# Lukeasargen/Show-Attend-and-Tell-Pytorch-Lightning

Hardware: AMD Instinct MI355X
Metric: captions/sec (train step) at B=128, 256px, seq_len=22 (higher is better)
Workload: dtype bf16; 1 GPU; C2: resnet50 encoder_size=7 encoder_dim=512 vocab=6400 T=22, 128 images/GPU x R=5 captions, trainable encoder, Adam, full lengths, decoder_tf=always; global_batch_images=128, parallelism=dp1, grad_bucket_dtype=fp32

## Files before the change

### include/sat_hip.h

```cpp
#ifndef SAT_HIP_H
#define SAT_HIP_H
#include <stddef.h>
#include <stdint.h>

#ifdef __cplusplus
extern "C" {
#endif

#define SAT_HIP_ABI_VERSION 23

int sat_abi_version(void);
int sat_debug_trace_launches(int32_t on);
int sat_debug_option(const char* name, int32_t value);
const char* sat_last_error(void);

typedef struct sat_profile_entry {
    char name[96];
    int64_t launches;
    double total_ms;
    double flops;
    double bytes;
} sat_profile_entry;
int sat_profile_start(void);
int sat_profile_start_only(const char* name);
int sat_profile_pause(int32_t paused);
int sat_profile_stop(sat_profile_entry* out, int32_t max_entries, int32_t* n_out);

typedef struct sat_gemm_desc {
    const float* A; int64_t lda; const int32_t* a_rows;
    const float* B; int64_t ldb;
    float* C; int64_t ldc;       const int32_t* c_rows;
    int32_t M, N, K;
    int32_t amode, bmode;
    int32_t accumulate;
    int32_t epi;
    const float* bias; const float* e0; int64_t lde0; int32_t c0, c1;
    float* slab; int64_t slab_elems;
} sat_gemm_desc;
int sat_gemm_f32(const sat_gemm_desc* d, void* stream);
typedef struct sat_gemm_types { int32_t a_bf16, b_bf16, c_bf16, bf16_mfma; } sat_gemm_types;
int sat_gemm_ex(const sat_gemm_desc* d, const sat_gemm_types* t, void* stream);

typedef struct sat_decoder_dims {
    int32_t B;
    int32_t R;
    int32_t T;
    int32_t L;
    int32_t D;
    int32_t A;
    int32_t m;
    int32_t n;
    int32_t V;
    int32_t P;
    int32_t deep_output;
    int32_t padding_idx;
    int32_t precision;
    int32_t layers;
    float embed_max_norm;
    float dropout;
    float embedding_dropout;
    uint64_t dropout_seed;
} sat_decoder_dims;

#define SAT_MAX_LSTM_LAYERS 4
typedef struct sat_decoder_params {
    float* embedding;
    float* init_f_w; float* init_f_b;
    float* init_i_w; float* init_i_b;
    float* w_ih; float* w_hh;
    float* b_ih; float* b_hh;
    float* att_enc;
    float* att_dec;
    float* att_f;
    float* beta_w; float* beta_b;
    float* out_hidden;
    float* out_context;
    float* out_w; float* out_b;
    float* up_w_ih[SAT_MAX_LSTM_LAYERS - 1]; float* up_w_hh[SAT_MAX_LSTM_LAYERS - 1];
    float* up_b_ih[SAT_MAX_LSTM_LAYERS - 1]; float* up_b_hh[SAT_MAX_LSTM_LAYERS - 1];
} sat_decoder_params;

typedef struct sat_decoder_batch {
    const float* ann;
    const int32_t* caps;
    const int32_t* lengths;
    const int32_t* prow;
    const int32_t* src_row;
    const int32_t* step_offsets_host;
    const int32_t* teacher_host;
} sat_decoder_batch;

size_t sat_decoder_workspace_bytes(const sat_decoder_dims* d);

int sat_decoder_train_fwd(const sat_decoder_dims* d, const sat_decoder_params* w, const sat_decoder_batch* b,
                          float* logits_packed, float* alphas, void* workspace, size_t workspace_bytes, void* stream);

int sat_decoder_train_bwd(const sat_decoder_dims* d, const sat_decoder_params* w, const sat_decoder_batch* b,
                          const float* dlogits_packed, const float* alphas , const float* dalphas,
                          const sat_decoder_params* g, float* dann, void* workspace, size_t workspace_bytes, void* stream);

int sat_ce_label_smooth_fwd(const float* logits, const int32_t* targets, int32_t P, int32_t V, float smoothing,
                            float* lse_rows, float* loss_rows, int32_t* correct_rows, float* out, void* stream);
int sat_ce_label_smooth_bwd(const float* logits, const int32_t* targets, const float* lse_rows, int32_t P, int32_t V,
                            float smoothing, const float* gscale, float* dlogits, void* stream);
int sat_doubly_stochastic_fwd(const float* alphas, int32_t N, int32_t T1, int32_t L, float gamma,
                              float* asum, float* part, float* out, void* stream);
int sat_doubly_stochastic_bwd(const float* asum, const float* gscale, int32_t N, int32_t T1, int32_t L, float gamma,
                              float* dalphas, void* stream);

#define SAT_TEMPERATURE_MAX 8
size_t sat_temperature_workspace_bytes(int32_t P, int32_t V);
int sat_temperature_nll(const float* logits, const int32_t* targets, int32_t P, int32_t V, const float* temperatures,
                        int32_t n_temperatures, float* loss_out, float* grad_out, void* workspace, void* stream);
int sat_temperature_fit(const float* logits, const int32_t* targets, int32_t P, int32_t V, float init, float lr, float momentum,
                        int32_t nesterov, int32_t iters, float* t_trace, float* loss_trace, void* workspace, void* stream);

size_t sat_decoder_infer_workspace_bytes(const sat_decoder_dims* d, int32_t max_beams);
int sat_decoder_infer_begin(const sat_decoder_dims* d, const sat_decoder_params* w, const float* ann , int32_t beams,
                            int32_t max_beams, float* h , float* c, void* workspace, size_t workspace_bytes, void* stream);
int sat_decoder_infer_step(const sat_decoder_dims* d, const sat_decoder_params* w, const float* ann, const int32_t* tokens, int32_t beams,
                           int32_t max_beams, float* h, float* c, float* logits , float* alpha ,
                           const float* h_noise ,
                           void* workspace, size_t workspace_bytes, void* stream);
size_t sat_beam_search_workspace_bytes(const sat_decoder_dims* d, int32_t beamk);
int sat_beam_search_batched(const sat_decoder_dims* d, const sat_decoder_params* w, const float* ann , int32_t beamk,
                            int32_t max_gen_length, const float* temperatures_host, int32_t n_temperatures, const int32_t* special_ids_host,
                            int32_t* tok_in, int32_t* prev_row, float* alpha_hist, int32_t* fin_count, int32_t* fin_step, int32_t* fin_row,
                            float* fin_score, float* fin_mean, void* workspace, size_t workspace_bytes, void* stream);
#define SAT_SAMPLE_BEAM 0
#define SAT_SAMPLE_MULTINOMIAL 1
#define SAT_SAMPLE_TOPK 2
#define SAT_SAMPLE_NUCLEUS 3
typedef struct sat_beam_sampling {
    int32_t method;
    int32_t sample_topk;
    uint64_t seed;
    const float* gumbel;
    float decoder_noise;
    float sample_topp;
    const float* normals;
} sat_beam_sampling;
int sat_beam_search_sampled(const sat_decoder_dims* d, const sat_decoder_params* w, const float* ann, int32_t beamk, int32_t max_gen_length,
                            const float* temperatures_host, int32_t n_temperatures, const int32_t* special_ids_host, const sat_beam_sampling* sampling,
                            int32_t* tok_in, int32_t* prev_row, float* alpha_hist, int32_t* fin_count, int32_t* fin_step, int32_t* fin_row,
                            float* fin_score, float* fin_mean, void* workspace, size_t workspace_bytes, void* stream);
typedef struct sat_beam_constraints {
    int32_t topg;
    int32_t max_prefix;
    const int32_t* prefix;
    const int32_t* prefix_len;
    const int32_t* banned;
    int32_t n_banned;
    int32_t reserved;
} sat_beam_constraints;
size_t sat_beam_search_constrained_workspace_bytes(const sat_decoder_dims* d, int32_t beamk, int32_t topg);
int sat_beam_search_constrained(const sat_decoder_dims* d, const sat_decoder_params* w, const float* ann, int32_t beamk, int32_t max_gen_length,
                                const float* temperatures_host, int32_t n_temperatures, const int32_t* special_ids_host, const sat_beam_sampling* sampling,
                                const sat_beam_constraints* constraints, int32_t* tok_in, int32_t* prev_row, float* alpha_hist, int32_t* fin_count,
                                int32_t* fin_step, int32_t* fin_row, float* fin_score, float* fin_mean, void* workspace, size_t workspace_bytes,
                                void* stream);
int sat_beam_scores(const float* logits, int32_t beams, int32_t V, float temperature, const int32_t* masked_ids ,
                    int32_t n_masked, const float* parent_scores , float* scores, void* stream);
int sat_topk(const float* x, float* work , int64_t n, int32_t k, float* values, int32_t* indices, void* stream);
int sat_nucleus_keys(const float* scores, int32_t rows, int32_t V, float topp, float step, uint64_t seed, uint64_t stream,
                     const float* gumbel , float* keys, int32_t* nucleus_size , void* stream_handle);

#define SAT_CAPTION_MAX_LEN 128
#define SAT_CAPTION_MAX_REFS 16
#define SAT_CAPTION_MAX_EMBED 2048
#define SAT_RESCORE_NONE 0
#define SAT_RESCORE_LN 1
#define SAT_RESCORE_WR 2
#define SAT_RESCORE_BAR 3
int sat_beam_select(const int32_t* tok_in, const int32_t* prev_row, const int32_t* fin_count, const int32_t* fin_step, const int32_t* fin_row,
                    const float* fin_score, const float* fin_mean, const float* alpha_hist , int32_t B, int32_t beamk,
                    int32_t max_gen_length, int32_t L, int32_t rescore_method, float rescore_reward, int32_t pad_id, int32_t* cap_tokens,
                    int32_t* cap_len, float* cap_score, float* cap_raw, int32_t* cap_step, float* cap_alpha , void* stream);
int sat_caption_stats(const int32_t* cap_tokens, const int32_t* cap_len, int32_t cap_width, const int32_t* refs, const int32_t* ref_lengths,
                      int32_t B, int32_t R, int32_t T, int32_t* stats, void* stream);
int sat_caption_cosine(const int32_t* cap_tokens, const int32_t* cap_len, int32_t cap_width, const int32_t* refs, const int32_t* ref_lengths,
                       int32_t B, int32_t R, int32_t T, const float* embedding, int32_t V, int32_t m, float* best_cosine, void* stream);

#define SAT_NGRAM_TABLE_MAX_CAPACITY (1LL << 36)
size_t sat_ngram_table_bytes(int64_t capacity);
int sat_ngram_table_clear(void* table, int64_t capacity, void* stream);
int sat_ngram_table_add(const int32_t* refs, const int32_t* ref_lengths, int32_t B, int32_t R, int32_t T, void* table, int64_t capacity,
                        int32_t* error_flag, void* stream);
// ... 304 lines not shown
```

### show-attend-and-tell-pytorch-lightning_amd/_lib.py

```python
import ctypes as C
import weakref
import os

import torch

_HERE = os.path.dirname(os.path.abspath(__file__))
LIB_PATH = os.path.join(_HERE, "libsat_hip.so")
_lib = None

f32p = C.POINTER(C.c_float)
i32p = C.POINTER(C.c_int32)


class GemmDesc(C.Structure):
    _fields_ = [("A", C.c_void_p), ("lda", C.c_int64), ("a_rows", C.c_void_p),
                ("B", C.c_void_p), ("ldb", C.c_int64),
                ("C", C.c_void_p), ("ldc", C.c_int64), ("c_rows", C.c_void_p),
                ("M", C.c_int32), ("N", C.c_int32), ("K", C.c_int32),
                ("amode", C.c_int32), ("bmode", C.c_int32), ("accumulate", C.c_int32), ("epi", C.c_int32),
                ("bias", C.c_void_p), ("e0", C.c_void_p), ("lde0", C.c_int64), ("c0", C.c_int32), ("c1", C.c_int32),
                ("slab", C.c_void_p), ("slab_elems", C.c_int64)]


class DecoderDims(C.Structure):
# ... 30 lines not shown
class DecoderParams(C.Structure):
    _fields_ = [(k, C.c_void_p) for k in PARAM_FIELDS] + [(k, C.c_void_p * (MAX_LSTM_LAYERS - 1)) for k in UP_FIELDS]


class OptTensor(C.Structure):
    _fields_ = [("p", C.c_void_p), ("g", C.c_void_p), ("m", C.c_void_p), ("v", C.c_void_p), ("n", C.c_int64), ("lr", C.c_float),
                ("weight_decay", C.c_float), ("shadow_bf16", C.c_void_p)]


class OptHyper(C.Structure):
    _fields_ = [("kind", C.c_int32), ("nesterov", C.c_int32), ("first_step", C.c_int32), ("beta1", C.c_float), ("beta2", C.c_float),
                ("eps", C.c_float), ("bias_correction1", C.c_float), ("bias_correction2_sqrt", C.c_float), ("momentum", C.c_float),
                ("clip_value", C.c_float)]


class BeamSampling(C.Structure):
    _fields_ = [("method", C.c_int32), ("sample_topk", C.c_int32), ("seed", C.c_uint64), ("gumbel", C.c_void_p), ("decoder_noise", C.c_float),
                ("sample_topp", C.c_float), ("normals", C.c_void_p)]


SAMPLE_METHODS = {"beam": 0, "multinomial": 1, "topk": 2, "nucleus": 3}


class BeamConstraints(C.Structure):
    _fields_ = [("topg", C.c_int32), ("max_prefix", C.c_int32), ("prefix", C.c_void_p), ("prefix_len", C.c_void_p), ("banned", C.c_void_p),
                ("n_banned", C.c_int32), ("reserved", C.c_int32)]


class ImageDesc(C.Structure):
    _fields_ = [("offset", C.c_int64)] + [(k, C.c_int32) for k in ("height", "width", "crop_top", "crop_left", "crop_h", "crop_w", "resized_h",
                                                                  "resized_w", "out_top", "out_left", "flip", "reserved")]


class ImageJitter(C.Structure):
    _fields_ = [("order", C.c_int32 * 4), ("brightness", C.c_float), ("contrast", C.c_float), ("saturation", C.c_float), ("hue_shift", C.c_int32)]


class ImageWarp(C.Structure):
    _fields_ = [("kind", C.c_int32), ("reserved", C.c_int32), ("coeffs", C.c_double * 8)]


class JpegDesc(C.Structure):
    _fields_ = [(k, C.c_int64) for k in ("data_offset", "data_bytes", "segments_offset", "out_offset", "block_offset")] + \
               [(k, C.c_int32) for k in ("height", "width", "components", "h_samp", "v_samp", "restart_interval", "n_segments", "segment_base")] + \
               [(k, C.c_int32 * 3) for k in ("quant", "dc_table", "ac_table")] + [("reserved", C.c_int32)]


class JpegDecodeOpts(C.Structure):
    _fields_ = [("subseq_bytes", C.c_int32), ("reserved", C.c_int32), ("parallel_min_bytes", C.c_int64), ("info", C.c_void_p)]


class JpegScan(C.Structure):
    _fields_ = [(k, C.c_int64) for k in ("data_offset", "data_bytes", "segments_offset")] + \
               [("picture", C.c_int32), ("level", C.c_int32), ("n_components", C.c_int32), ("component", C.c_int32 * 3)] + \
               [(k, C.c_int32) for k in ("ss", "se", "ah", "al")] + [("dc_table", C.c_int32 * 3), ("ac_table", C.c_int32)] + \
               [(k, C.c_int32) for k in ("restart_interval", "n_segments", "segment_base", "reserved")]


class JpegQTable(C.Structure):
    _fields_ = [("q", C.c_uint16 * 64)]


class JpegHTable(C.Structure):
    _fields_ = [("lookup", C.c_uint16 * 512), ("maxcode", C.c_int32 * 18), ("valoffset", C.c_int32 * 18), ("huffval", C.c_uint8 * 256)]


class DecoderBatch(C.Structure):
    _fields_ = [("ann", C.c_void_p), ("caps", C.c_void_p), ("lengths", C.c_void_p), ("prow", C.c_void_p), ("src_row", C.c_void_p),
                ("step_offsets_host", C.c_void_p), ("teacher_host", C.c_void_p)]


SYMBOLS = {
    "sat_abi_version": (C.c_int, []),
    "sat_debug_trace_launches": (C.c_int, [C.c_int32]),
    "sat_debug_option": (C.c_int, [C.c_char_p, C.c_int32]),
    "sat_last_error": (C.c_char_p, []),
    "sat_gemm_f32": (C.c_int, [C.POINTER(GemmDesc), C.c_void_p]),
    "sat_decoder_workspace_bytes": (C.c_size_t, [C.POINTER(DecoderDims)]),
    "sat_decoder_train_fwd": (C.c_int, [C.POINTER(DecoderDims), C.POINTER(DecoderParams), C.POINTER(DecoderBatch),
                                        C.c_void_p, C.c_void_p, C.c_void_p, C.c_size_t, C.c_void_p]),
    "sat_decoder_train_bwd": (C.c_int, [C.POINTER(DecoderDims), C.POINTER(DecoderParams), C.POINTER(DecoderBatch),
                                        C.c_void_p, C.c_void_p, C.c_void_p, C.POINTER(DecoderParams), C.c_void_p,
                                        C.c_void_p, C.c_size_t, C.c_void_p]),
    "sat_ce_label_smooth_fwd": (C.c_int, [C.c_void_p, C.c_void_p, C.c_int32, C.c_int32, C.c_float, C.c_void_p, C.c_void_p,
                                          C.c_void_p, C.c_void_p, C.c_void_p]),
    "sat_ce_label_smooth_bwd": (C.c_int, [C.c_void_p, C.c_void_p, C.c_void_p, C.c_int32, C.c_int32, C.c_float, C.c_void_p,
                                          C.c_void_p, C.c_void_p]),
    "sat_doubly_stochastic_fwd": (C.c_int, [C.c_void_p, C.c_int32, C.c_int32, C.c_int32, C.c_float, C.c_void_p, C.c_void_p,
                                            C.c_void_p, C.c_void_p]),
    "sat_doubly_stochastic_bwd": (C.c_int, [C.c_void_p, C.c_void_p, C.c_int32, C.c_int32, C.c_int32, C.c_float, C.c_void_p, C.c_void_p]),
    "sat_attention_precompute": (C.c_int, [C.c_void_p, C.c_void_p, C.c_void_p, C.c_int32, C.c_int32, C.c_int32, C.c_int32, C.c_void_p]),
    "sat_attention_step_fwd": (C.c_int, [C.c_void_p, C.c_void_p, C.c_void_p, C.c_int32, C.c_void_p, C.c_void_p, C.c_int32,
                                         C.c_void_p, C.c_int32, C.c_void_p, C.c_void_p, C.c_int32, C.c_int32, C.c_int32,
                                         C.c_int32, C.c_int32, C.c_void_p]),
}


class GemmTypes(C.Structure):
    _fields_ = [(k, C.c_int32) for k in ("a_bf16", "b_bf16", "c_bf16", "bf16_mfma")]


class ConvGeom(C.Structure):
    _fields_ = [(k, C.c_int32) for k in ("N", "H", "W", "C", "K", "R", "S", "stride", "pad", "stride_w")]


class BlockDesc(C.Structure):
    _fields_ = ([(k, C.c_int32) for k in ("kind", "stride", "cin", "mid", "cout", "has_ds", "N", "H", "W", "fwd_res_bn", "dgrad_join", "bn_bwd_epilogue")] +
                [(k, C.c_void_p) for k in ("w1", "w2", "w3", "wd")] +
                [("gamma", C.c_void_p * 4), ("beta", C.c_void_p * 4), ("running_mean", C.c_void_p * 4), ("running_var", C.c_void_p * 4),
                 ("eps", C.c_float * 4), ("momentum", C.c_float * 4)] +
                [(k, C.c_void_p) for k in ("dw1", "dw2", "dw3", "dwd")] + [("dgamma", C.c_void_p * 4), ("dbeta", C.c_void_p * 4)])


_vp, _i32, _i64, _f = C.c_void_p, C.c_int32, C.c_int64, C.c_float
SYMBOLS.update({
    "sat_encoder_blocks_arena_bytes": (C.c_size_t, [C.POINTER(BlockDesc), _i32]),
    "sat_encoder_blocks_fwd": (C.c_int, [C.POINTER(BlockDesc), _i32, _vp, _vp, C.c_size_t, _vp, C.POINTER(C.c_void_p), _vp]),
    "sat_encoder_blocks_bwd": (C.c_int, [C.POINTER(BlockDesc), _i32, _i32, _i32, _vp, _vp, C.c_size_t, _vp, _vp, _i32, _vp, _vp, _i64, _vp, _i64, _vp, _vp,
                                         C.POINTER(C.c_void_p), C.POINTER(C.c_void_p), C.POINTER(C.c_int32), _vp]),
    "sat_conv2d_fwd": (C.c_int, [_vp, _vp, _vp, _vp, C.POINTER(ConvGeom), _vp]),
    "sat_conv2d_dgrad": (C.c_int, [_vp, _vp, _vp, C.POINTER(ConvGeom), _i32, _vp]),
    "sat_conv2d_wgrad": (C.c_int, [_vp, _vp, _vp, C.POINTER(ConvGeom), _vp, _i64, _vp]),
    "sat_conv2d_wgrad_slab_bytes": (C.c_size_t, [C.POINTER(ConvGeom)]),
    "sat_conv2d_fwd_bf16": (C.c_int, [_vp, _vp, _vp, _vp, C.POINTER(ConvGeom), _vp]),
    "sat_conv2d_dgrad_bf16": (C.c_int, [_vp, _vp, _vp, C.POINTER(ConvGeom), _i32, _vp]),
    "sat_conv2d_wgrad_bf16": (C.c_int, [_vp, _vp, _vp, C.POINTER(ConvGeom), _vp, _i64, _vp]),
    "sat_gemm_ex": (C.c_int, [C.POINTER(GemmDesc), C.POINTER(GemmTypes), _vp]),
    "sat_image_normalize_nhwc4": (C.c_int, [_vp, _vp, _i32, _i32, _i32, C.POINTER(C.c_float), C.POINTER(C.c_float), _vp]),
    "sat_pad_channels_3to4": (C.c_int, [_vp, _vp, _i64, _i32, _vp]),
    "sat_bn_scratch_bytes": (C.c_size_t, [_i64, _i32]),
    "sat_bn_train_fwd": (C.c_int, [_vp, _i64, _i32, _vp, _vp, _f, _f, _vp, _vp, _vp, _vp, _vp, _i32, _vp, _vp, _vp]),
    "sat_bn_eval_fwd": (C.c_int, [_vp, _i64, _i32, _vp, _vp, _f, _vp, _vp, _vp, _i32, _vp, _vp]),
    "sat_colsum": (C.c_int, [_vp, _i64, _i64, _i32, _vp, _vp, _vp]),
    "sat_bn_train_bwd": (C.c_int, [_vp, _vp, _vp, _i64, _i32, _vp, _vp, _vp, _i32, _vp, _vp, _vp, _vp, _i32, _vp, _vp]),
    "sat_bn_train_fwd_t": (C.c_int, [_i32, _vp, _i64, _i32, _vp, _vp, _f, _f, _vp, _vp, _vp, _vp, _vp, _i32, _vp, _vp, _vp, _vp]),
    "sat_conv2d_fwd_stats_bytes": (C.c_size_t, [C.POINTER(ConvGeom)]),
    "sat_conv2d_fwd_bf16_stats": (C.c_int, [_vp, _vp, _vp, C.POINTER(ConvGeom), _vp, C.POINTER(C.c_int32), _vp]),
    "sat_bn_train_fwd_tiles_bf16": (C.c_int, [_vp, _i64, _i32, _vp, _i32, _vp, _vp, _f, _f, _vp, _vp, _vp, _vp, _vp, _i32, _vp, _vp, _vp, _vp]),
    "sat_bn_eval_fwd_t": (C.c_int, [_i32, _vp, _i64, _i32, _vp, _vp, _f, _vp, _vp, _vp, _i32, _vp, _vp]),
    "sat_conv2d_dgrad_stats_bytes": (C.c_size_t, [C.POINTER(ConvGeom)]),
    "sat_conv2d_dgrad_bf16_bnstats": (C.c_int, [_vp, _vp, _vp, C.POINTER(ConvGeom), _i32, _vp, _vp, _vp, _vp, _vp, C.POINTER(C.c_int32), _vp]),
    "sat_bn_train_fwd_tiles_bf16_resbn": (C.c_int, [_vp, _i64, _i32, _vp, _i32, _vp, _vp, C.c_float, C.c_float, _vp, _vp, _vp, _vp, _vp, _vp, _vp, _vp, _vp,
                                                   _i32, _vp, _vp, _vp, _vp]),
    "sat_conv2d_dgrad_bf16_fused": (C.c_int, [_vp, _vp, _vp, C.POINTER(ConvGeom), _vp, _vp, _vp, _vp, _vp, _vp, _vp, C.POINTER(C.c_int32), _vp]),
    "sat_bn_train_bwd_tiles_bf16": (C.c_int, [_vp, _vp, _i64, _i32, _vp, _i32, _vp, _vp, _vp, _i32, _vp, _vp, _vp, _vp, _i32, _vp, _vp, _vp]),
    "sat_bn_train_bwd_t": (C.c_int, [_i32, _vp, _vp, _vp, _i64, _i32, _vp, _vp, _vp, _i32, _vp, _vp, _vp, _vp, _i32, _vp, _vp, _vp]),
    "sat_maxpool3x3s2_fwd_t": (C.c_int, [_i32, _vp, _vp, _vp, _i32, _i32, _i32, _i32, _vp]),
    "sat_maxpool3x3s2_bwd_t": (C.c_int, [_i32, _vp, _vp, _vp, _i32, _i32, _i32, _i32, _vp]),
    "sat_cast_f32_to_bf16": (C.c_int, [_vp, _vp, _i64, _vp]),
    "sat_image_normalize_nhwc8_bf16": (C.c_int, [_vp, _vp, _i32, _i32, _i32, C.POINTER(C.c_float), C.POINTER(C.c_float), _vp]),
    "sat_image_normalize_nhwc4_padded_bf16": (C.c_int, [_vp, _vp, _i32, _i32, _i32, C.POINTER(C.c_float), C.POINTER(C.c_float), _vp]),
    "sat_stem_filter_pairs": (C.c_int, [_vp, _vp, _i32, _vp]),
    "sat_dwconv3x3_fwd_t": (C.c_int, [_i32, _vp, _vp, _vp, _i32, _i32, _i32, _i32, _i32, _vp]),
    "sat_dwconv3x3_dgrad_t": (C.c_int, [_i32, _vp, _vp, _vp, _i32, _i32, _i32, _i32, _i32, _vp]),
    "sat_dwconv3x3_wgrad_scratch_bytes": (C.c_size_t, [_i32, _i32, _i32, _i32, _i32]),
    "sat_dwconv3x3_wgrad_t": (C.c_int, [_i32, _vp, _vp, _vp, _i32, _i32, _i32, _i32, _i32, _vp, _vp]),
    "sat_dwconv3x3_plan": (C.c_int, [_i32, _i32, _i32, _i32, _i32, _i32, _i32, C.POINTER(_i32)]),
    "sat_shuffle_join_t": (C.c_int, [_i32, _vp, _vp, _vp, _vp, _vp, _i64, _i32, _i32, _vp]),
    "sat_shuffle_split_t": (C.c_int, [_i32, _vp, _vp, _vp, _vp, _vp, _i64, _i32, _i32, _vp]),
    "sat_cast_bf16_to_f32": (C.c_int, [_vp, _vp, _i64, _vp]),
    "sat_grouped_filter_expand": (C.c_int, [_vp, _vp, _i32, _i32, _i32, _i32, _i32, _vp]),
    "sat_grouped_filter_grad_extract": (C.c_int, [_vp, _vp, _i32, _i32, _i32, _i32, _vp]),
    "sat_stem_filter_grad_unpairs": (C.c_int, [_vp, _vp, _i32, _vp]),
    "sat_stem_filter_pad": (C.c_int, [_vp, _vp, _i64, _vp]),
    "sat_stem_filter_grad_unpad": (C.c_int, [_vp, _vp, _i64, _vp]),
    "sat_maxpool3x3s2_fwd": (C.c_int, [_vp, _vp, _vp, _i32, _i32, _i32, _i32, _vp]),
# ... 201 lines not shown
```

### show-attend-and-tell-pytorch-lightning_amd/csrc/api.hip

```cpp
#include <stdarg.h>

#include "../../include/sat_hip.h"
#include "decoder.h"
#include "gemm.h"
#include "gemm_bf16_common.h"
#include "temperature.h"
#include "caption_score.h"

namespace sat {
static thread_local char g_err[512] = {0};
int& dev_switch(int which) {
    static int v[SW_COUNT] = {0 , getenv("SAT_NO_WGRAD3X3") ? !atoi(getenv("SAT_NO_WGRAD3X3")) : 1,
                              getenv("SAT_REDUCE_Z16") ? atoi(getenv("SAT_REDUCE_Z16")) : 1, getenv("SAT_WIDE_TILES") ? atoi(getenv("SAT_WIDE_TILES")) : 0,
                              getenv("SAT_BN_ONEPASS") ? atoi(getenv("SAT_BN_ONEPASS")) : 1,
                              getenv("SAT_BN_VPT") ? atoi(getenv("SAT_BN_VPT")) : 2,
                              getenv("SAT_ACC_PREFETCH") ? atoi(getenv("SAT_ACC_PREFETCH")) : 0};
    return v[which];
}
int& trace_launches() { static int on = getenv("SAT_TRACE_LAUNCH") ? 1 : 0; return on; }
char* last_error_buf() { return g_err; }
int fail(int code, const char* fmt, ...) {
    va_list ap; va_start(ap, fmt); vsnprintf(g_err, sizeof g_err, fmt, ap); va_end(ap);
    return code;
}
}

using namespace sat;

extern "C" {

int sat_abi_version(void) { return SAT_HIP_ABI_VERSION; }
int sat_debug_trace_launches(int32_t on) { sat::trace_launches() = on ? 1 : 0; return SAT_OK; }
int sat_debug_option(const char* name, int32_t value) {
    if (!name) return fail(SAT_EINVAL, "debug_option: null name");
    if (!strcmp(name, "wgrad3x3")) { dev_switch(SW_WGRAD3X3) = value; return SAT_OK; }
    if (!strcmp(name, "reduce_z16")) { dev_switch(SW_REDUCE_Z16) = value; return SAT_OK; }
    if (!strcmp(name, "acc_prefetch")) { dev_switch(SW_ACC_PREFETCH) = value; return SAT_OK; }
    if (!strcmp(name, "bn_vpt")) { dev_switch(SW_BN_VPT) = value; return SAT_OK; }
    if (!strcmp(name, "bn_onepass")) { dev_switch(SW_BN_ONEPASS) = value; return SAT_OK; }
    if (!strcmp(name, "wide_tiles")) { dev_switch(SW_WIDE_TILES) = value; return SAT_OK; }
    if (!strcmp(name, "glds_tile")) { glds_force_tile() = value; return SAT_OK; }
    if (!strcmp(name, "glds_stages8")) { glds_stages8() = value; return SAT_OK; }
    if (!strcmp(name, "glds_tall_k")) { glds_tall_k() = value; return SAT_OK; }
    if (!strcmp(name, "glds_tall_conv")) { glds_tall_conv() = value; return SAT_OK; }
    if (!strcmp(name, "tile_override")) { gemm_tile_override() = value; return SAT_OK; }
    return fail(SAT_EINVAL, "debug_option: unknown option %s", name);
}
const char* sat_last_error(void) { return last_error_buf(); }

static int gemm_from_desc(const sat_gemm_desc* d, const sat_gemm_types* t, void* stream);
int sat_gemm_f32(const sat_gemm_desc* d, void* stream) { return gemm_from_desc(d, nullptr, stream); }
int sat_gemm_ex(const sat_gemm_desc* d, const sat_gemm_types* t, void* stream) {
    if (!t) return fail(SAT_EINVAL, "sat_gemm_ex: null type descriptor");
    return gemm_from_desc(d, t, stream);
}
static int gemm_from_desc(const sat_gemm_desc* d, const sat_gemm_types* t, void* stream) {
    if (!d) return fail(SAT_EINVAL, "sat_gemm_f32: null descriptor");
    if (d->amode != A_ROW && d->amode != A_KMAJOR) return fail(SAT_EINVAL, "sat_gemm_f32: amode %d (dense modes only)", d->amode);
    if (d->bmode != B_ROW && d->bmode != B_KMAJOR) return fail(SAT_EINVAL, "sat_gemm_f32: bmode %d (dense modes only)", d->bmode);
    GemmArgs g;
    g.A = d->A; g.lda = d->lda; g.a_rows = d->a_rows; g.B = d->B; g.ldb = d->ldb; g.C = d->C; g.ldc = d->ldc; g.c_rows = d->c_rows;
    g.M = d->M; g.N = d->N; g.K = d->K; g.amode = d->amode; g.bmode = d->bmode; g.accumulate = d->accumulate; g.epi = d->epi;
    g.bias = d->bias; g.e0 = d->e0; g.lde0 = d->lde0; g.c0 = d->c0; g.c1 = d->c1; g.slab = d->slab; g.slab_elems = d->slab_elems;
    if (t) { g.a_bf16 = t->a_bf16; g.b_bf16 = t->b_bf16; g.c_bf16 = t->c_bf16; g.bf16_mfma = t->bf16_mfma; }
    return launch_gemm(g, (hipStream_t)stream);
}

size_t sat_decoder_workspace_bytes(const sat_decoder_dims* d) {
    if (check_dims(d) != SAT_OK) return 0;
    return decoder_workspace_bytes(*d);
}

static int check_params(const sat_decoder_dims* d, const sat_decoder_params* w, const char* what) {
    if (!w) return fail(SAT_EINVAL, "%s: null parameter struct", what);
    if (!w->embedding || !w->init_f_w || !w->init_f_b || !w->init_i_w || !w->init_i_b || !w->w_ih || !w->w_hh || !w->b_ih || !w->b_hh ||
        !w->att_enc || !w->att_dec || !w->att_f || !w->beta_w || !w->beta_b || !w->out_hidden || !w->out_w)
        return fail(SAT_EINVAL, "%s: null tensor in parameter struct", what);
    if (d->deep_output && !w->out_context) return fail(SAT_EINVAL, "%s: deep output needs output.context.weight", what);
    for (int l = 1; l < d->layers; ++l)
        if (!w->up_w_ih[l - 1] || !w->up_w_hh[l - 1] || !w->up_b_ih[l - 1] || !w->up_b_hh[l - 1])
            return fail(SAT_EINVAL, "%s: null tensor for LSTM layer %d", what, l);
    return SAT_OK;
}
static int check_batch(const sat_decoder_batch* b) {
    if (!b || !b->ann || !b->caps || !b->lengths || !b->prow || !b->src_row || !b->step_offsets_host || !b->teacher_host)
        return fail(SAT_EINVAL, "decoder: null field in batch struct");
    return SAT_OK;
}

int sat_decoder_train_fwd(const sat_decoder_dims* d, const sat_decoder_params* w, const sat_decoder_batch* b, float* logits_packed,
                          float* alphas, void* workspace, size_t workspace_bytes, void* stream) {
    SAT_TRY(check_dims(d)); SAT_TRY(check_params(d, w, "decoder_train_fwd")); SAT_TRY(check_batch(b));
    if (!alphas || !workspace || (d->P > 0 && !logits_packed)) return fail(SAT_EINVAL, "decoder_train_fwd: null output/workspace");
    return decoder_fwd(*d, *w, *b, logits_packed, alphas, (char*)workspace, workspace_bytes, (hipStream_t)stream);
}

int sat_decoder_train_bwd(const sat_decoder_dims* d, const sat_decoder_params* w, const sat_decoder_batch* b, const float* dlogits_packed,
                          const float* alphas, const float* dalphas, const sat_decoder_params* g, float* dann, void* workspace,
                          size_t workspace_bytes, void* stream) {
    SAT_TRY(check_dims(d)); SAT_TRY(check_params(d, w, "decoder_train_bwd")); SAT_TRY(check_params(d, g, "decoder_train_bwd(grads)")); SAT_TRY(check_batch(b));
    if (!alphas || !dann || !workspace || (d->P > 0 && !dlogits_packed)) return fail(SAT_EINVAL, "decoder_train_bwd: null input/output/workspace");
    return decoder_bwd(*d, *w, *b, dlogits_packed, alphas, dalphas, *g, dann, (char*)workspace, workspace_bytes, (hipStream_t)stream);
}

int sat_ce_label_smooth_fwd(const float* logits, const int32_t* targets, int32_t P, int32_t V, float smoothing, float* lse_rows,
                            float* loss_rows, int32_t* correct_rows, float* out, void* stream) {
    if (!logits || !targets || !lse_rows || !loss_rows || !correct_rows || !out) return fail(SAT_EINVAL, "ce_label_smooth_fwd: null pointer");
    return ce_fwd(logits, targets, P, V, smoothing, lse_rows, loss_rows, correct_rows, out, (hipStream_t)stream);
}
int sat_ce_label_smooth_bwd(const float* logits, const int32_t* targets, const float* lse_rows, int32_t P, int32_t V, float smoothing,
                            const float* gscale, float* dlogits, void* stream) {
    if (!logits || !targets || !lse_rows || !dlogits) return fail(SAT_EINVAL, "ce_label_smooth_bwd: null pointer");
    return ce_bwd(logits, targets, lse_rows, P, V, smoothing, gscale, dlogits, (hipStream_t)stream);
}
int sat_doubly_stochastic_fwd(const float* alphas, int32_t N, int32_t T1, int32_t L, float gamma, float* asum, float* part, float* out, void* stream) {
    if (!alphas || !asum || !part || !out) return fail(SAT_EINVAL, "doubly_stochastic_fwd: null pointer");
    return ds_fwd(alphas, N, T1, L, gamma, asum, part, out, (hipStream_t)stream);
}
int sat_doubly_stochastic_bwd(const float* asum, const float* gscale, int32_t N, int32_t T1, int32_t L, float gamma, float* dalphas, void* stream) {
    if (!asum || !dalphas) return fail(SAT_EINVAL, "doubly_stochastic_bwd: null pointer");
    return ds_bwd(asum, gscale, N, T1, L, gamma, dalphas, (hipStream_t)stream);
}

size_t sat_temperature_workspace_bytes(int32_t P, int32_t V) {
    if (P <= 0 || V <= 0) { fail(SAT_EINVAL, "temperature_workspace_bytes: non-positive size (P=%d V=%d)", P, V); return 0; }
    return temperature_workspace_bytes(P, V);
}
int sat_temperature_nll(const float* logits, const int32_t* targets, int32_t P, int32_t V, const float* temperatures, int32_t n_temperatures,
                        float* loss_out, float* grad_out, void* workspace, void* stream) {
    if (!logits || !targets || !temperatures || !loss_out || !grad_out || !workspace) return fail(SAT_EINVAL, "temperature_nll: null pointer");
    if (P <= 0 || V <= 0) return fail(SAT_EINVAL, "temperature_nll: empty input (P=%d V=%d)", P, V);
    if (n_temperatures < 1 || n_temperatures > SAT_TEMPERATURE_MAX)
        return fail(SAT_EINVAL, "temperature_nll: %d temperatures (1..%d in one pass)", n_temperatures, SAT_TEMPERATURE_MAX);
    if ((uintptr_t)workspace % 16) return fail(SAT_EINVAL, "temperature_nll: workspace must be 16-byte aligned");
    return temperature_nll(logits, targets, P, V, temperatures, n_temperatures, loss_out, grad_out, (char*)workspace, (hipStream_t)stream);
}
int sat_temperature_fit(const float* logits, const int32_t* targets, int32_t P, int32_t V, float init, float lr, float momentum, int32_t nesterov,
                        int32_t iters, float* t_trace, float* loss_trace, void* workspace, void* stream) {
    if (!logits || !targets || !t_trace || !loss_trace || !workspace) return fail(SAT_EINVAL, "temperature_fit: null pointer");
    if (P <= 0 || V <= 0 || iters <= 0) return fail(SAT_EINVAL, "temperature_fit: non-positive size (P=%d V=%d iters=%d)", P, V, iters);
    if (!(init > 0.f) || !(init < INFINITY)) return fail(SAT_EINVAL, "temperature_fit: initial temperature %g is not a positive finite number", init);
    if (!(lr > 0.f)) return fail(SAT_EINVAL, "temperature_fit: learning rate %g is not positive", lr);
    if (!(momentum >= 0.f)) return fail(SAT_EINVAL, "temperature_fit: momentum %g is negative", momentum);
    if ((uintptr_t)workspace % 16) return fail(SAT_EINVAL, "temperature_fit: workspace must be 16-byte aligned");
    return temperature_fit(logits, targets, P, V, init, lr, momentum, nesterov ? 1 : 0, iters, t_trace, loss_trace, (char*)workspace, (hipStream_t)stream);
}

size_t sat_decoder_infer_workspace_bytes(const sat_decoder_dims* d, int32_t max_beams) {
    if (check_dims(d) != SAT_OK || max_beams < 1) return 0;
    return decoder_infer_workspace_bytes(*d, max_beams);
}
int sat_decoder_infer_begin(const sat_decoder_dims* d, const sat_decoder_params* w, const float* ann, int32_t beams, int32_t max_beams,
                            float* h, float* c, void* workspace, size_t workspace_bytes, void* stream) {
    SAT_TRY(check_dims(d)); SAT_TRY(check_params(d, w, "decoder_infer_begin"));
    if (!ann || !h || !c || !workspace) return fail(SAT_EINVAL, "decoder_infer_begin: null pointer");
    return decoder_infer_begin(*d, *w, ann, beams, max_beams, h, c, (char*)workspace, workspace_bytes, (hipStream_t)stream);
}
int sat_decoder_infer_step(const sat_decoder_dims* d, const sat_decoder_params* w, const float* ann, const int32_t* tokens, int32_t beams,
                           int32_t max_beams, float* h, float* c, float* logits, float* alpha, const float* h_noise, void* workspace,
                           size_t workspace_bytes, void* stream) {
    SAT_TRY(check_dims(d)); SAT_TRY(check_params(d, w, "decoder_infer_step"));
    if (!ann || !tokens || !h || !c || !logits || !alpha || !workspace) return fail(SAT_EINVAL, "decoder_infer_step: null pointer");
    return decoder_infer_step(*d, *w, ann, tokens, beams, max_beams, h, c, logits, alpha, h_noise, (char*)workspace, workspace_bytes, (hipStream_t)stream);
}
size_t sat_beam_search_workspace_bytes(const sat_decoder_dims* d, int32_t beamk) {
    if (check_dims(d) != SAT_OK || beamk < 1) return 0;
    return decoder_beam_workspace_bytes(*d, beamk);
}
int sat_beam_search_batched(const sat_decoder_dims* d, const sat_decoder_params* w, const float* ann, int32_t beamk, int32_t max_gen_length,
                            const float* temperatures_host, int32_t n_temperatures, const int32_t* special_ids_host, int32_t* tok_in, int32_t* prev_row,
                            float* alpha_hist, int32_t* fin_count, int32_t* fin_step, int32_t* fin_row, float* fin_score, float* fin_mean, void* workspace,
                            size_t workspace_bytes, void* stream) {
    SAT_TRY(check_dims(d)); SAT_TRY(check_params(d, w, "beam_search_batched"));
    if (!ann || !temperatures_host || !special_ids_host || !tok_in || !prev_row || !alpha_hist || !fin_count || !fin_step || !fin_row || !fin_score || !fin_mean || !workspace)
        return fail(SAT_EINVAL, "beam_search_batched: null pointer");
    for (int i = 0; i < n_temperatures; ++i) if (!(temperatures_host[i] > 0.f)) return fail(SAT_EINVAL, "beam_search_batched: temperature %g", temperatures_host[i]);
    return decoder_beam_batched(*d, *w, ann, beamk, max_gen_length, temperatures_host, n_temperatures, special_ids_host, tok_in, prev_row, alpha_hist, fin_count,
                                fin_step, fin_row, fin_score, fin_mean, (char*)workspace, workspace_bytes, (hipStream_t)stream, nullptr);
}
int sat_beam_search_sampled(const sat_decoder_dims* d, const sat_decoder_params* w, const float* ann, int32_t beamk, int32_t max_gen_length,
                            const float* temperatures_host, int32_t n_temperatures, const int32_t* special_ids_host, const sat_beam_sampling* sampling,
                            int32_t* tok_in, int32_t* prev_row, float* alpha_hist, int32_t* fin_count, int32_t* fin_step, int32_t* fin_row, float* fin_score,
                            float* fin_mean, void* workspace, size_t workspace_bytes, void* stream) {
    SAT_TRY(check_dims(d)); SAT_TRY(check_params(d, w, "beam_search_sampled"));
    if (!ann || !temperatures_host || !special_ids_host || !tok_in || !prev_row || !alpha_hist || !fin_count || !fin_step || !fin_row || !fin_score || !fin_mean || !workspace)
        return fail(SAT_EINVAL, "beam_search_sampled: null pointer");
    for (int i = 0; i < n_temperatures; ++i) if (!(temperatures_host[i] > 0.f)) return fail(SAT_EINVAL, "beam_search_sampled: temperature %g", temperatures_host[i]);
// ... 244 lines not shown
```

### show-attend-and-tell-pytorch-lightning_amd/csrc/decoder.h

```cpp
#pragma once
#include "../../include/sat_hip.h"
#include "common.h"

namespace sat {
struct Ws;
int check_dims(const sat_decoder_dims* d);
size_t decoder_workspace_bytes(const sat_decoder_dims& d);
int decoder_fwd(const sat_decoder_dims& d, const sat_decoder_params& p, const sat_decoder_batch& b, float* logits, float* alphas,
                char* ws, size_t ws_bytes, hipStream_t st);
int decoder_bwd(const sat_decoder_dims& d, const sat_decoder_params& p, const sat_decoder_batch& b, const float* dlogits,
                const float* alphas, const float* dalphas, const sat_decoder_params& g, float* dann, char* ws, size_t ws_bytes, hipStream_t st);
enum { ATT_OP_FWD = 0, ATT_OP_BWD = 1, ATT_OP_CONTEXT_BWD = 2 };
enum { ATT_FORM_SPLIT = 0, ATT_FORM_SINGLE = 1 };
enum : unsigned { ATT_HAS_SCRATCH = 1, ATT_ANN_ALIGNED = 2, ATT_ROWS_ALIGNED = 4, ATT_HAS_BF16 = 8 };
struct AttPlan {
    int form = 0, rn = 0, passes = 0;
    int vw = 0, dchunk = 0;
    int nq = 0, lq = 0;
    size_t lds0 = 0, lds1 = 0;
};
int attention_plan(int op, int R, int L, int D, int A, int hc_ld, int T1, unsigned flags, AttPlan& plan, const char* who);
int launch_attention_fwd(hipStream_t st, const float* ann, const float* U, const float* hc, int hc_ld, const float* wf,
                         const int* lengths, int step, float* alphas, int T1, float* Z, float* XZ, int B, int R, int L, int D, int A, float* sc = nullptr, void* xzb = nullptr,
                         const void* annb = nullptr);
size_t decoder_infer_workspace_bytes(const sat_decoder_dims& d, int Kmax);
int decoder_infer_begin(const sat_decoder_dims& d, const sat_decoder_params& p, const float* ann, int K, int Kmax, float* h, float* c,
                        char* ws, size_t ws_bytes, hipStream_t st);
int decoder_infer_step(const sat_decoder_dims& d, const sat_decoder_params& p, const float* ann, const int* tokens, int K, int Kmax,
                       float* h, float* c, float* logits, float* alpha, const float* h_noise, char* ws, size_t ws_bytes, hipStream_t st);
size_t decoder_beam_workspace_bytes(const sat_decoder_dims& d, int K, int topg = 0);
int decoder_beam_batched(const sat_decoder_dims& d, const sat_decoder_params& p, const float* ann, int K, int max_gen_length, const float* temps_host,
                         int n_temps, const int* special_host, int* tok_in, int* prev_row, float* alpha_hist, int* fin_count, int* fin_step, int* fin_row,
                         float* fin_score, float* fin_mean, char* ws, size_t ws_bytes, hipStream_t st, const sat_beam_sampling* sampling,
                         const sat_beam_constraints* constraints = nullptr);
int launch_attention_bwd(hipStream_t st, const float* ann, const float* U, const float* hc, int hc_ld, const float* wf, const int* lengths, int step,
                         const float* alphas, const float* dalphas, int T1, const float* Z, const float* dZ, const float* dXZ, float* DZ, float* dhc,
                         int dhc_ld, float* dU, float* dwf_part, float* da, int B, int R, int L, int D, int A, void* dhcb = nullptr, const void* annb = nullptr);
int attention_context_bwd(const float* alphas, const float* DZ, const int* lengths, float* dann, int accumulate, int B, int R, int T1, int L, int D, hipStream_t st);
int lstm_cell_fwd(const float* x, int in, const float* h_prev, const float* c_prev, const float* w_ih, const float* w_hh, const float* b_ih, const float* b_hh,
                  float* gates, float* h_new, float* c_new, float* bias_scratch, int N, int n, hipStream_t st);
int lstm_cell_bwd(const float* x, int in, const float* h_prev, const float* c_prev, const float* c_new, const float* gates, const float* dh_new, const float* dc_new,
                  const float* w_ih, const float* w_hh, float* dx, float* dh_prev, float* dc_prev, float* dw_ih, float* dw_hh, float* db_ih, float* db_hh,
                  float* dgates, float* scratch, int N, int n, hipStream_t st);
int deep_output_fwd(const float* prev_embed, const float* hidden, const float* context, const float* w_hidden, const float* w_context, const float* w_out,
                    const float* b_out, float dropout, unsigned long long seed, float* u, float* udrop, float* logits, int N, int m, int n, int D, int V, hipStream_t st);
int deep_output_bwd(const float* dlogits, const float* hidden, const float* context, const float* u, const float* udrop, const float* w_hidden, const float* w_context,
                    const float* w_out, float dropout, unsigned long long seed, float* d_prev_embed, float* d_hidden, float* d_context, float* dw_hidden,
                    float* dw_context, float* dw_out, float* db_out, float* scratch, int N, int m, int n, int D, int V, hipStream_t st);
int init_lstm_fwd(const float* ann, const float* w_f, const float* b_f, const float* w_i, const float* b_i, float dropout, unsigned long long seed, float* mean,
                  float* f, float* init, int N, int L, int D, int m, int n2, hipStream_t st);
int init_lstm_bwd(const float* dinit, const float* mean, const float* f, const float* w_f, const float* w_i, float dropout, unsigned long long seed, float* dw_f,
                  float* db_f, float* dw_i, float* db_i, float* dann, float* df, float* dmean, float* scratch, int N, int L, int D, int m, int n2, hipStream_t st);
int embedding_fwd(float* table, const int* tokens, float* out, int rows, int V, int m, float max_norm, int* flags, hipStream_t st);
int embedding_bwd(const float* dY, const int* tokens, float* dtable, int rows, int V, int m, int padding_idx, int* scratch, hipStream_t st);
int sigmoid_bwd(const float* dy, const float* y, float* dpre, long n, hipStream_t st);
int beam_scores(const float* logits, int K, int V, float temperature, const int* masked, int n_masked, const float* parent, float* scores, hipStream_t st);
int topk(const float* x, float* work, long n, int k, float* values, int* indices, hipStream_t st);
int nucleus_keys(const float* scores, int rows, int V, float topp, float step, unsigned long long seed, unsigned long long stream, const float* gumbel,
                 float* keys, int* nucleus_size, hipStream_t st);
int colsum_public(const float* x, long ld, long rows, int cols, float* out, float* scratch, hipStream_t st);
int ce_fwd(const float* logits, const int* targets, int P, int V, float smoothing, float* lse_rows, float* loss_rows, int* correct_rows, float* out, hipStream_t st);
int ce_bwd(const float* logits, const int* targets, const float* lse_rows, int P, int V, float smoothing, const float* gscale, float* dlogits, hipStream_t st);
int ds_fwd(const float* alphas, int N, int T1, int L, float gamma, float* asum, float* part, float* out, hipStream_t st);
int ds_bwd(const float* asum, const float* gscale, int N, int T1, int L, float gamma, float* dalphas, hipStream_t st);
}
```

### show-attend-and-tell-pytorch-lightning_amd/csrc/decoder.hip

```cpp
#include "../../include/sat_hip.h"
#include <stdlib.h>
#include "decoder.h"
#include "profile.h"
#include "decoder_kernels.h"
#include "gemm.h"

namespace sat {

struct Ws {
    size_t total = 0;
    float *U, *mean, *f, *init_img, *H_all, *C_all, *HC, *Z, *XZ, *Y, *GY, *Uact, *Wcat, *bcat;
    float *Udrop, *mean_rows, *f_rows, *init_rows, *df_rows;
    float *GU, *DGU, *bup;
    __bf16 *Wb_out, *Ub;
    __bf16 *annb;
    __bf16 *Hb, *XZb, *Wcat_b, *Wz_b, *DHCb;
    int* Tok; int* flags;
    int *emb_count, *emb_offset, *emb_cursor, *emb_list;
    float *SC, *DA;
    float *dA, *dHout, *dZout, *DZ, *DHC, *dXZ, *dHc, *dCc, *dU, *dwf_part, *dY, *colpart, *dinit_img, *df, *dmean, *slab;
    char *zero_begin, *zero_end;
    long slab_elems;
};

Ws layout(const sat_decoder_dims& d, char* base) {
    Ws w; size_t off = 0;
    const long N = (long)d.B * d.R, T1 = d.T - 1, HCW = d.A + d.D + 4L * d.n;
    auto take = [&](size_t elems, size_t esz = 4) { size_t o = off; off += (elems * esz + 255) & ~(size_t)255; return base ? base + o : (char*)nullptr; };
    w.U = (float*)take((size_t)d.B * d.L * d.A);
    w.mean = (float*)take((size_t)d.B * d.D);
    w.f = (float*)take((size_t)d.B * d.m);
    const int NL = d.layers;
    w.init_img = (float*)take((size_t)d.B * 2 * d.n * NL);
    w.H_all = (float*)take((size_t)NL * (T1 + 1) * N * d.n);
    w.C_all = (float*)take((size_t)NL * (T1 + 1) * N * d.n);
    w.GU = w.DGU = w.bup = nullptr;
    if (NL > 1) {
        w.GU = (float*)take((size_t)(NL - 1) * T1 * N * 4 * d.n); w.DGU = (float*)take((size_t)(NL - 1) * T1 * N * 4 * d.n);
        w.bup = (float*)take((size_t)(NL - 1) * 4 * d.n);
    }
    w.HC = (float*)take((size_t)T1 * N * HCW);
    w.Z = (float*)take((size_t)T1 * N * d.D);
    w.XZ = (float*)take((size_t)T1 * N * d.D);
    w.Y = (float*)take((size_t)T1 * N * d.m);
    w.GY = (float*)take((size_t)T1 * N * 4 * d.n);
    w.Uact = (float*)take((size_t)(d.P > 0 ? d.P : 1) * d.m);
    w.Wcat = (float*)take((size_t)HCW * d.n);
    w.bcat = (float*)take((size_t)HCW);
    w.Tok = (int*)take((size_t)T1 * N);
    w.Udrop = w.mean_rows = w.f_rows = w.init_rows = w.df_rows = nullptr;
    if (d.dropout > 0.f) {
        w.Udrop = (float*)take((size_t)(d.P > 0 ? d.P : 1) * d.m); w.mean_rows = (float*)take((size_t)N * d.D); w.f_rows = (float*)take((size_t)N * d.m);
        w.init_rows = (float*)take((size_t)N * 2 * d.n * NL); w.df_rows = (float*)take((size_t)N * d.m);
    }
    w.Wb_out = w.Ub = nullptr;
    if (d.precision && d.m % 64 == 0 && d.V % 8 == 0) {
        w.Wb_out = (__bf16*)take((size_t)d.V * d.m, 2); w.Ub = (__bf16*)take((size_t)(d.P > 0 ? d.P : 1) * d.m, 2);
    }
    w.Hb = w.XZb = w.Wcat_b = w.Wz_b = w.DHCb = nullptr;
    w.annb = (d.precision && d.D % 4 == 0 && d.A % 4 == 0) ? (__bf16*)take((size_t)d.B * d.L * d.D, 2) : nullptr;
    if (d.precision && d.layers == 1 && d.n % 64 == 0 && d.D % 64 == 0 && d.A % 4 == 0 && d.m % 4 == 0) {
        w.Hb = (__bf16*)take((size_t)(T1 + 1) * N * d.n, 2); w.XZb = (__bf16*)take((size_t)N * d.D, 2);
        w.Wcat_b = (__bf16*)take((size_t)HCW * d.n, 2); w.Wz_b = (__bf16*)take((size_t)4 * d.n * d.D, 2);
        w.DHCb = (__bf16*)take((size_t)N * HCW, 2);
    }
    w.flags = (int*)take((size_t)d.V);
    w.emb_count = (int*)take((size_t)d.V); w.emb_offset = (int*)take((size_t)d.V + 1); w.emb_cursor = (int*)take((size_t)d.V);
    w.emb_list = (int*)take((size_t)T1 * N);
    w.SC = (float*)take((size_t)N * d.L); w.DA = (float*)take((size_t)N * d.L);
    w.dA = (float*)take((size_t)(d.P > 0 ? d.P : 1) * d.m);
    w.DZ = (float*)take((size_t)T1 * N * d.D);
    w.DHC = (float*)take((size_t)T1 * N * HCW);
    w.dXZ = (float*)take((size_t)N * d.D);
    w.dHout = (float*)take((size_t)T1 * N * d.n); w.zero_begin = (char*)w.dHout;
    w.dZout = (float*)take((size_t)T1 * N * d.D);
    w.dHc = (float*)take((size_t)NL * N * d.n);
    w.dCc = (float*)take((size_t)NL * N * d.n);
    w.dU = (float*)take((size_t)d.B * d.L * d.A);
    w.dwf_part = (float*)take((size_t)d.B * d.A);
    w.zero_end = base ? base + off : (char*)nullptr;
    w.dY = (float*)take((size_t)T1 * N * d.m);
    long maxrows = d.P > T1 * N ? d.P : T1 * N; if (maxrows < d.B * (long)d.L) maxrows = d.B * (long)d.L;
    long maxcols = d.V > HCW ? d.V : HCW;
    w.colpart = (float*)take((size_t)cdiv(maxrows, 256) * maxcols);
    w.dinit_img = (float*)take((size_t)d.B * 2 * d.n * NL);
    w.df = (float*)take((size_t)d.B * d.m);
    w.dmean = (float*)take((size_t)d.B * d.D);
    w.slab_elems = 8L << 20;
    w.slab = (float*)take((size_t)w.slab_elems);
    w.total = off;
    return w;
}

int check_dims(const sat_decoder_dims* d) {
    SAT_REQUIRE(d, "decoder: null dims");
    SAT_REQUIRE(d->B > 0 && d->R > 0 && d->T >= 2 && d->L > 0 && d->D > 0 && d->A > 0 && d->m > 0 && d->n > 0 && d->V > 0,
                "decoder: non-positive dimension (B=%d R=%d T=%d L=%d D=%d A=%d m=%d n=%d V=%d)", d->B, d->R, d->T, d->L, d->D, d->A, d->m, d->n, d->V);
    SAT_REQUIRE(d->P >= 0 && (long)d->P <= (long)d->B * d->R * (d->T - 1), "decoder: packed token count %d out of range", d->P);
    SAT_REQUIRE(d->layers >= 1 && d->layers <= SAT_MAX_LSTM_LAYERS, "decoder: layers=%d outside 1..%d", d->layers, SAT_MAX_LSTM_LAYERS);
    SAT_REQUIRE(d->dropout >= 0.f && d->dropout < 1.f && d->embedding_dropout >= 0.f && d->embedding_dropout < 1.f, "decoder: dropout must lie in [0,1)");
    return SAT_OK;
}

static thread_local int t_bf16_mfma = 0;
static int gemm(hipStream_t st, int amode, int bmode, const float* A, long lda, const float* B, long ldb, float* C, long ldc,
                int M, int N, int K, int acc = 0, int epi = EPI_NONE, const float* bias = nullptr, const int* a_rows = nullptr,
                const int* c_rows = nullptr, const float* e0 = nullptr, long lde0 = 0, int c0 = 0, int c1 = 0, float* slab = nullptr, long slab_elems = 0) {
    GemmArgs g;
    g.A = A; g.lda = lda; g.B = B; g.ldb = ldb; g.C = C; g.ldc = ldc; g.M = M; g.N = N; g.K = K;
    g.amode = amode; g.bmode = bmode; g.accumulate = acc; g.epi = epi; g.bias = bias; g.a_rows = a_rows; g.c_rows = c_rows;
    g.e0 = e0; g.lde0 = lde0; g.c0 = c0; g.c1 = c1; g.slab = slab; g.slab_elems = slab_elems;
    g.bf16_mfma = t_bf16_mfma;
    return launch_gemm(g, st);
}

static int cast_bf16(hipStream_t st, const float* src, __bf16* dst, long n) {
    hipLaunchKernelGGL(cast_bf16_kernel, dim3(cdiv(n / 4, 256)), dim3(256), 0, st, src, dst, n / 4);
    return launch_ok("cast_bf16");
}
static int gemm_bb_nt(hipStream_t st, const __bf16* A, long lda, const __bf16* B, long ldb, float* C, long ldc, int M, int N, int K, int epi, const float* bias,
                      int acc = 0, int c0 = 0, int c1 = 0) {
    GemmArgs g;
    g.A = A; g.lda = lda; g.B = B; g.ldb = ldb; g.C = C; g.ldc = ldc; g.M = M; g.N = N; g.K = K;
    g.amode = A_ROW; g.bmode = B_ROW; g.epi = epi; g.bias = bias; g.a_bf16 = g.b_bf16 = 1; g.c_bf16 = 0; g.bf16_mfma = 1;
    g.accumulate = acc; g.c0 = c0; g.c1 = c1;
    return launch_gemm(g, st);
}

static int gemm_bb_nn(hipStream_t st, const __bf16* A, long lda, const __bf16* B, long ldb, float* C, long ldc, int M, int N, int K, int acc, float* slab, long slab_elems) {
    GemmArgs g;
    g.A = A; g.lda = lda; g.B = B; g.ldb = ldb; g.C = C; g.ldc = ldc; g.M = M; g.N = N; g.K = K;
    g.amode = A_ROW; g.bmode = B_KMAJOR; g.a_bf16 = g.b_bf16 = 1; g.c_bf16 = 0; g.bf16_mfma = 1; g.accumulate = acc; g.slab = slab; g.slab_elems = slab_elems;
    return launch_gemm(g, st);
}

static int colsum(hipStream_t st, const Ws& w, const float* x, long ld, int rows, int cols, float* out, int accumulate = 0, float scale = 1.f) {
    if (cols <= 0) return SAT_OK;
    if (rows <= 0) { if (!accumulate) SAT_TRY(dev_fill_bytes(st, out, 0, (size_t)cols * 4)); return SAT_OK; }
    int nparts = cdiv(rows, 256);
    if (cols % 4 == 0 && ld % 4 == 0 && (reinterpret_cast<uintptr_t>(x) & 15) == 0)
        hipLaunchKernelGGL(colsum_part4_kernel, dim3(cdiv(cols / 4, 128), nparts), dim3(128), 0, st, x, ld, rows, cols / 4, 256, w.colpart);
    else
        hipLaunchKernelGGL(colsum_part_kernel, dim3(cdiv(cols, 256), nparts), dim3(256), 0, st, x, ld, rows, cols, 256, w.colpart);
    SAT_TRY(launch_ok("colsum_part"));
    hipLaunchKernelGGL(colsum_finish_kernel, dim3(cdiv(cols, 256)), dim3(256), 0, st, w.colpart, nparts, cols, out, accumulate, scale);
    return launch_ok("colsum_finish");
}

static int live_steps(const sat_decoder_dims& d, const sat_decoder_batch& b) {
    const int T1 = d.T - 1; int ts = 0;
    for (int t = 0; t < T1; ++t) if (b.step_offsets_host[t + 1] > b.step_offsets_host[t]) ts = t + 1;
    return ts;
}

static size_t att_fwd_lds(int L, int A, int vw) { return (size_t)(ATT_RMAX * L + ATT_RMAX * A + A + ATT_RMAX * ATT_THREADS * vw) * 4; }
static size_t att_bwd_lds(int L, int A, int D) { return (size_t)(2 * ATT_RMAX * L + ATT_RMAX * A + A + ATT_RMAX * D + ATTB_WAVES * ATT_RMAX * A + ATTB_WAVES * A) * 4; }

int attention_plan(int op, int R, int L, int D, int A, int hc_ld, int T1, unsigned flags, AttPlan& p, const char* who) {
    p = AttPlan();
    SAT_REQUIRE(op >= ATT_OP_FWD && op <= ATT_OP_CONTEXT_BWD, "%s: op=%d (0 forward, 1 backward, 2 context backward)", who, op);
    SAT_REQUIRE(R >= 1 && L >= 1 && D >= 1 && T1 >= 1 && (op == ATT_OP_CONTEXT_BWD || (A >= 1 && hc_ld >= A + D)),
                "%s: bad shape (R=%d L=%d D=%d A=%d hc_ld=%d T1=%d)", who, R, L, D, A, hc_ld, T1);
    const bool scratch = flags & ATT_HAS_SCRATCH, ann_al = flags & ATT_ANN_ALIGNED, rows_al = flags & ATT_ROWS_ALIGNED;
    p.rn = R < ATT_RMAX ? R : ATT_RMAX;
    p.passes = cdiv(R, p.rn);
    const int RN = p.rn;
    if (op == ATT_OP_FWD) {
        if (scratch && D % 4 == 0 && A % 4 == 0 && hc_ld % 4 == 0 && ann_al && rows_al) {
            p.form = ATT_FORM_SPLIT; p.vw = 4; p.dchunk = ATTC_DCH;
            p.lds0 = (size_t)(RN * A + A) * 4;
            p.lds1 = (size_t)((RN * L + 3) & ~3) * 4 + (size_t)16 * RN * 16 * 16;
        } else {
            p.form = ATT_FORM_SINGLE;
            const bool vec = D % 4 == 0 && ann_al;
            p.vw = vec ? 4 : 1;
            p.dchunk = vec ? 256 : 64;
            if (p.dchunk > D) p.dchunk = D;
            p.lds0 = att_fwd_lds(L, A, p.vw);
        }
    } else if (op == ATT_OP_BWD) {
        if (scratch && D % 4 == 0 && ann_al) {
            p.form = ATT_FORM_SPLIT; p.vw = 4;
            p.lds0 = (size_t)RN * D * 4;
            p.lds1 = (size_t)(RN * L + RN * ATTB_KCH + 32 * (RN + 1) * ATTB_KCH) * 4;
        } else {
            p.form = ATT_FORM_SINGLE; p.vw = 1;
            p.lds0 = att_bwd_lds(L, A, D);
        }
    } else {
        const int lq4 = (L + 3) / 4;
        p.form = ATT_FORM_SINGLE; p.rn = R; p.passes = 1; p.vw = 1;
        p.nq = (lq4 <= 13) ? 13 : 16;
        p.lq = (lq4 + p.nq - 1) / p.nq * p.nq;
        p.lds0 = (size_t)R * T1 * p.lq * 16;
    }
    if ((flags & ATT_HAS_BF16) && p.form != ATT_FORM_SPLIT) { p = AttPlan(); SAT_REQUIRE(false, "%s: the bf16 copies need the split kernels (aligned shapes)", who); }
    if (p.lds0 > 160 * 1024 || p.lds1 > 160 * 1024) {
        const size_t need = p.lds0 > p.lds1 ? p.lds0 : p.lds1;
        p = AttPlan();
        SAT_REQUIRE(false, "%s: R=%d L=%d D=%d A=%d T1=%d need %zu B of LDS (> 160 KiB)", who, R, L, D, A, T1, need);
    }
    return SAT_OK;
}
static bool al16(const void* p) { return (reinterpret_cast<uintptr_t>(p) & 15) == 0; }
static bool al8(const void* p) { return (reinterpret_cast<uintptr_t>(p) & 7) == 0; }

static bool ann_bf16_enabled() { static const bool off = getenv("SAT_ANN_BF16") && !atoi(getenv("SAT_ANN_BF16")); return !off; }
static bool attention_split_enabled() {
    static const int no_split = getenv("SAT_ATT_FUSED") ? atoi(getenv("SAT_ATT_FUSED")) : 0;
    return !no_split;
}
template <int RN, typename TA>
static int attention_fwd_split(hipStream_t st, const TA* ann, const float* U, const float* hc, int hc_ld, const float* wf, const int* lengths, int step,
                               float* alphas, int T1, float* Z, float* XZ, int B, int R, int L, int D, int A, float* sc, __bf16* xzb, const AttPlan& pl) {
    const size_t lds_s = pl.lds0, lds_c = pl.lds1;
// ... 165 lines not shown

    SAT_TRY(gemm(st, A_ROW, B_ROW, b.ann, D, p.att_enc, D, w.U, A, d.B * d.L, A, D));
    hipLaunchKernelGGL(ann_mean_kernel, dim3(d.B), dim3(256), 0, st, b.ann, w.mean, d.L, D);
    SAT_TRY(launch_ok("ann_mean"));
    if (d.dropout > 0.f) {
        hipLaunchKernelGGL(init_mean_rows_kernel, dim3(cdiv((long)N * D, 256)), dim3(256), 0, st, w.mean, w.mean_rows, N, d.R, D, d.dropout, (unsigned long long)d.dropout_seed);
        SAT_TRY(launch_ok("init_mean_rows"));
        SAT_TRY(gemm(st, A_ROW, B_ROW, w.mean_rows, D, p.init_f_w, D, w.f_rows, m, N, m, D, 0, EPI_BIAS, p.init_f_b));
        SAT_TRY(gemm(st, A_ROW, B_ROW, w.f_rows, m, p.init_i_w, m, w.init_rows, 2 * n * NL, N, 2 * n * NL, m, 0, EPI_BIAS, p.init_i_b));
        for (int l = 0; l < NL; ++l) {
            SAT_TRY(dev_copy_bytes(st, Hs(0, l), w.init_rows + (long)l * N * n, (size_t)N * n * 4));
            SAT_TRY(dev_copy_bytes(st, Cs(0, l), w.init_rows + (long)(NL + l) * N * n, (size_t)N * n * 4));
        }
    } else {
        SAT_TRY(gemm(st, A_ROW, B_ROW, w.mean, D, p.init_f_w, D, w.f, m, d.B, m, D, 0, EPI_BIAS, p.init_f_b));
        SAT_TRY(gemm(st, A_ROW, B_ROW, w.f, m, p.init_i_w, m, w.init_img, 2 * n * NL, d.B, 2 * n * NL, m, 0, EPI_BIAS, p.init_i_b));
        hipLaunchKernelGGL(init_expand_kernel, dim3(cdiv(2L * NL * N * n, 256)), dim3(256), 0, st, w.init_img, w.H_all, w.C_all, N, d.R, n, NL, LS);
        SAT_TRY(launch_ok("init_expand"));
    }

    const __bf16* annb = (w.annb && attention_split_enabled() && ann_bf16_enabled() && al16(b.ann)) ? w.annb : nullptr;
    if (annb) SAT_TRY(cast_bf16(st, b.ann, w.annb, (long)d.B * d.L * D));
    if (use_b) {
        hipLaunchKernelGGL(cast_block_bf16_kernel, dim3(cdiv((long)4 * n * (D / 4), 256)), dim3(256), 0, st, p.w_ih + m, (long)(m + D), w.Wz_b, 4 * n, D);
        SAT_TRY(launch_ok("cast W_ih[:, m:]"));
        SAT_TRY(cast_bf16(st, Hs(0, 0), w.Hb, (long)N * n));
    }
    if (ts < T1) SAT_TRY(dev_fill_bytes(st, alphas, 0, (size_t)N * T1 * d.L * 4));

    SAT_TRY(dev_fill_bytes(st, w.Tok, 0xFF, (size_t)T1 * N * 4));
    for (int t = 0; t < ts;) {
        if (!b.teacher_host[t]) { ++t; continue; }
        int t1 = t + 1;
        while (t1 < ts && b.teacher_host[t1]) ++t1;
        hipLaunchKernelGGL(teacher_tokens_kernel, dim3(cdiv(N, 256), t1 - t), dim3(256), 0, st, b.caps, b.lengths, w.Tok + (long)t * N, N, d.T, t);
        SAT_TRY(launch_ok("teacher_tokens"));
        t = t1;
    }
    auto renorm = [&](const int* tok, int count) -> int {
        if (!(d.embed_max_norm > 0.f)) return SAT_OK;
        hipLaunchKernelGGL(embedding_mark_kernel, dim3(cdiv(count, 256)), dim3(256), 0, st, tok, count, w.flags, d.V);
        SAT_TRY(launch_ok("embedding_mark"));
        hipLaunchKernelGGL(embedding_renorm_kernel, dim3(d.V), dim3(64), 0, st, p.embedding, w.flags, m, d.embed_max_norm);
        return launch_ok("embedding_renorm");
    };
    if (d.embed_max_norm > 0.f) SAT_TRY(dev_fill_bytes(st, w.flags, 0, (size_t)d.V * 4));
    if (ts > 0) {
        SAT_TRY(renorm(w.Tok, ts * N));
        hipLaunchKernelGGL(gather_rows_kernel, dim3(ts * N), dim3(64), 0, st, p.embedding, w.Tok, w.Y, ts * N, m, d.embedding_dropout, (unsigned long long)d.dropout_seed, 0L);
        SAT_TRY(launch_ok("embedding gather"));
        SAT_TRY(gemm(st, A_ROW, B_ROW, w.Y, m, p.w_ih, m + D, w.GY, 4 * n, ts * N, 4 * n, m));
    }

    int pending = 0;
    for (int t = 0; t < ts; ++t) {
        float* hc = w.HC + (long)t * N * HCW;
        if (!b.teacher_host[t]) {
            SAT_TRY(flush_outputs(st, d, p, b, w, logits, b.step_offsets_host[pending], b.step_offsets_host[t]));
            pending = t;
            if (d.embed_max_norm > 0.f) {
                hipLaunchKernelGGL(argmax_tokens_kernel, dim3(N), dim3(256), 0, st, logits, b.prow + (long)(t - 1) * N, b.lengths, w.Tok + (long)t * N, d.V, t);
                SAT_TRY(launch_ok("argmax_tokens"));
                SAT_TRY(renorm(w.Tok + (long)t * N, N));
                hipLaunchKernelGGL(gather_rows_kernel, dim3(N), dim3(64), 0, st, p.embedding, w.Tok + (long)t * N, w.Y + (long)t * N * m, N, m, d.embedding_dropout, (unsigned long long)d.dropout_seed, (long)t * N);
                SAT_TRY(launch_ok("embedding gather"));
            } else {
                hipLaunchKernelGGL(argmax_gather_kernel, dim3(N), dim3(256), 0, st, logits, b.prow + (long)(t - 1) * N, b.lengths, w.Tok + (long)t * N, d.V, t, p.embedding,
                                   w.Y + (long)t * N * m, m, d.embedding_dropout, (unsigned long long)d.dropout_seed, (long)t * N);
                SAT_TRY(launch_ok("argmax + embedding gather"));
            }
            SAT_TRY(gemm(st, A_ROW, B_ROW, w.Y + (long)t * N * m, m, p.w_ih, m + D, w.GY + (long)t * N * 4 * n, 4 * n, N, 4 * n, m));
        }
        if (use_b) {
            SAT_TRY(gemm_bb_nt(st, w.Hb + (long)t * N * n, n, w.Wcat_b, n, hc, HCW, N, HCW, n, EPI_BIAS_SIGMOID_RANGE, w.bcat, 0, A, A + D));
        } else if (NL == 1) {
            SAT_TRY(gemm(st, A_ROW, B_ROW, Hs(t, 0), n, w.Wcat, n, hc, HCW, N, HCW, n, 0, EPI_BIAS_SIGMOID_RANGE, w.bcat,
                         nullptr, nullptr, nullptr, 0, A, A + D));
        } else {
            SAT_TRY(gemm(st, A_ROW, B_ROW, Hs(t, top), n, w.Wcat, n, hc, HCW, N, A + D, n, 0, EPI_BIAS_SIGMOID_RANGE, w.bcat,
                         nullptr, nullptr, nullptr, 0, A, A + D));
            SAT_TRY(gemm(st, A_ROW, B_ROW, Hs(t, 0), n, w.Wcat + (long)(A + D) * n, n, hc + A + D, HCW, N, 4 * n, n, 0, EPI_BIAS, w.bcat + A + D));
        }
        SAT_TRY(launch_attention_fwd(st, b.ann, w.U, hc, HCW, p.att_f, b.lengths, t, alphas, T1, w.Z + (long)t * N * D, w.XZ + (long)t * N * D,
                                     d.B, d.R, d.L, D, A, w.SC, use_b ? w.XZb : nullptr, annb));
        if (use_b) SAT_TRY(gemm_bb_nt(st, w.XZb, D, w.Wz_b, D, hc + A + D, HCW, N, 4 * n, D, EPI_NONE, nullptr, 1));
        else SAT_TRY(gemm(st, A_ROW, B_ROW, w.XZ + (long)t * N * D, D, p.w_ih + m, m + D, hc + A + D, HCW, N, 4 * n, D, 1));
        hipLaunchKernelGGL(lstm_cell_fwd_kernel, dim3(cdiv((long)N * n, 256)), dim3(256), 0, st, hc + A + D, HCW, w.GY + (long)t * N * 4 * n,
                           Cs(t, 0), Hs(t, 0), Cs(t + 1, 0), Hs(t + 1, 0), b.lengths, t, N, n, use_b ? w.Hb + (long)(t + 1) * N * n : (__bf16*)nullptr);
        SAT_TRY(launch_ok("lstm_cell_fwd"));
        for (int l = 1; l < NL; ++l) {
            float* gu = GUs(t, l);
            SAT_TRY(gemm(st, A_ROW, B_ROW, Hs(t + 1, l - 1), n, p.up_w_ih[l - 1], n, gu, 4 * n, N, 4 * n, n, 0, EPI_BIAS, w.bup + (long)(l - 1) * 4 * n));
            SAT_TRY(gemm(st, A_ROW, B_ROW, Hs(t, l), n, p.up_w_hh[l - 1], n, gu, 4 * n, N, 4 * n, n, 1));
            hipLaunchKernelGGL(lstm_cell_fwd_kernel, dim3(cdiv((long)N * n, 256)), dim3(256), 0, st, gu, 4 * n, (const float*)nullptr,
                               Cs(t, l), Hs(t, l), Cs(t + 1, l), Hs(t + 1, l), b.lengths, t, N, n);
            SAT_TRY(launch_ok("lstm_cell_fwd (stacked layer)"));
        }
    }
    return flush_outputs(st, d, p, b, w, logits, b.step_offsets_host[pending], b.step_offsets_host[ts]);
}

int decoder_bwd(const sat_decoder_dims& d, const sat_decoder_params& p, const sat_decoder_batch& b, const float* dlogits,
                       const float* alphas, const float* dalphas, const sat_decoder_params& g, float* dann, char* ws, size_t ws_bytes, hipStream_t st) {
    Ws w = layout(d, ws);
    t_bf16_mfma = d.precision ? 1 : 0;
    SAT_REQUIRE(ws_bytes >= w.total, "decoder_bwd: workspace %zu < %zu bytes", ws_bytes, w.total);
    const int N = d.B * d.R, T1 = d.T - 1, HCW = d.A + d.D + 4 * d.n, n = d.n, A = d.A, D = d.D, m = d.m, V = d.V, P = d.P;
    const int ts = live_steps(d, b);
    const int KR = ts * N;
    const int NL = d.layers, top = NL - 1;
    const long LS = (long)(T1 + 1) * N * n;
    auto Hs = [&](int t, int l) { return w.H_all + l * LS + (long)t * N * n; };
    auto Cs = [&](int t, int l) { return w.C_all + l * LS + (long)t * N * n; };
    auto GUs = [&](int t, int l) { return w.GU + ((long)(l - 1) * T1 + t) * N * 4 * n; };
    auto DGUs = [&](int t, int l) { return w.DGU + ((long)(l - 1) * T1 + t) * N * 4 * n; };
    auto dHcs = [&](int l) { return w.dHc + (long)l * N * n; };
    auto dCcs = [&](int l) { return w.dCc + (long)l * N * n; };
    float* const slab = w.slab; const long se = w.slab_elems;

    SAT_TRY(dev_fill_bytes(st, w.zero_begin, 0, (size_t)(w.zero_end - w.zero_begin)));
    if (NL > 1 && KR < T1 * N) SAT_TRY(dev_fill_bytes(st, w.DGU, 0, (size_t)(NL - 1) * T1 * N * 4 * n * 4));

    if (P > 0) {
        SAT_TRY(gemm(st, A_ROW, B_KMAJOR, dlogits, V, p.out_w, m, w.dA, m, P, m, V, 0, d.deep_output ? EPI_MUL_DTANH : EPI_NONE, nullptr,
                     nullptr, nullptr, w.Uact, m, 0, 0, slab, se));
        if (d.dropout > 0.f) {
            hipLaunchKernelGGL(dropout_rows_kernel, dim3(cdiv((long)P * m, 256)), dim3(256), 0, st, w.dA, w.dA, (long)P * m, m, d.dropout,
                               (unsigned long long)d.dropout_seed, 2u, 0L);
            SAT_TRY(launch_ok("output dropout bwd"));
        }
        SAT_TRY(gemm(st, A_KMAJOR, B_KMAJOR, dlogits, V, d.dropout > 0.f ? w.Udrop : w.Uact, m, g.out_w, m, V, m, P, 0, EPI_NONE, nullptr, nullptr, nullptr, nullptr, 0, 0, 0, slab, se));
        if (g.out_b) SAT_TRY(colsum(st, w, dlogits, V, P, V, g.out_b));
        SAT_TRY(gemm(st, A_ROW, B_KMAJOR, w.dA, m, p.out_hidden, n, w.dHout, n, P, n, m, 0, EPI_NONE, nullptr, nullptr, b.src_row));
        if (d.deep_output)
            SAT_TRY(gemm(st, A_ROW, B_KMAJOR, w.dA, m, p.out_context, D, w.dZout, D, P, D, m, 0, EPI_NONE, nullptr, nullptr, b.src_row));
    } else {
        SAT_TRY(dev_fill_bytes(st, g.out_w, 0, (size_t)V * m * 4));
        if (g.out_b) SAT_TRY(dev_fill_bytes(st, g.out_b, 0, (size_t)V * 4));
    }
    hipLaunchKernelGGL(scatter_rows_kernel, dim3(T1 * N), dim3(64), 0, st, w.dA, b.prow, w.dY, T1 * N, m);
    SAT_TRY(launch_ok("scatter dA"));
    const float* H1 = Hs(1, top);
    SAT_TRY(gemm(st, A_KMAJOR, B_KMAJOR, w.dY, m, H1, n, g.out_hidden, n, m, n, KR, 0, EPI_NONE, nullptr, nullptr, nullptr, nullptr, 0, 0, 0, slab, se));
    if (d.deep_output)
        SAT_TRY(gemm(st, A_KMAJOR, B_KMAJOR, w.dY, m, w.Z, D, g.out_context, D, m, D, KR, 0, EPI_NONE, nullptr, nullptr, nullptr, nullptr, 0, 0, 0, slab, se));
    else
        SAT_TRY(dev_fill_bytes(st, w.dY, 0, (size_t)T1 * N * m * 4));

    static const int att_fused = getenv("SAT_ATT_FUSED") ? atoi(getenv("SAT_ATT_FUSED")) : 0;
    const bool use_b = w.Hb != nullptr && !att_fused;
    const __bf16* annb = (w.annb && !att_fused && ann_bf16_enabled() && al16(b.ann)) ? w.annb : nullptr;
    for (int t = ts - 1; t >= 0; --t) {
        const float* hc = w.HC + (long)t * N * HCW;
        float* dhc = w.DHC + (long)t * N * HCW;
        for (int l = top; l >= 1; --l) {
            float* dgu = DGUs(t, l);
            hipLaunchKernelGGL(lstm_cell_bwd_kernel, dim3(cdiv((long)N * n, 256)), dim3(256), 0, st, GUs(t, l), 4 * n, Cs(t, l), Cs(t + 1, l),
                               l == top ? w.dHout + (long)t * N * n : (const float*)nullptr, dHcs(l), dCcs(l), dgu, 4 * n, b.lengths, t, N, n);
            SAT_TRY(launch_ok("lstm_cell_bwd (stacked layer)"));
            SAT_TRY(gemm(st, A_ROW, B_KMAJOR, dgu, 4 * n, p.up_w_ih[l - 1], n, dHcs(l - 1), n, N, n, 4 * n, 1, EPI_NONE, nullptr, nullptr, nullptr, nullptr, 0, 0, 0, slab, se));
            SAT_TRY(gemm(st, A_ROW, B_KMAJOR, dgu, 4 * n, p.up_w_hh[l - 1], n, dHcs(l), n, N, n, 4 * n, 1, EPI_NONE, nullptr, nullptr, nullptr, nullptr, 0, 0, 0, slab, se));
        }
        hipLaunchKernelGGL(lstm_cell_bwd_kernel, dim3(cdiv((long)N * n, 256)), dim3(256), 0, st, hc + A + D, HCW, Cs(t, 0),
                           Cs(t + 1, 0), top == 0 ? w.dHout + (long)t * N * n : (const float*)nullptr, dHcs(0), dCcs(0), dhc + A + D, HCW, b.lengths, t, N, n,
                           use_b ? w.DHCb + A + D : (__bf16*)nullptr);
        SAT_TRY(launch_ok("lstm_cell_bwd"));
        if (use_b) SAT_TRY(gemm_bb_nn(st, w.DHCb + A + D, HCW, w.Wz_b, D, w.dXZ, D, N, D, 4 * n, 0, slab, se));
        else SAT_TRY(gemm(st, A_ROW, B_KMAJOR, dhc + A + D, HCW, p.w_ih + m, m + D, w.dXZ, D, N, D, 4 * n, 0, EPI_NONE, nullptr, nullptr, nullptr, nullptr, 0, 0, 0, slab, se));
        SAT_TRY(launch_attention_bwd(st, b.ann, w.U, hc, HCW, p.att_f, b.lengths, t, alphas, dalphas, T1, w.Z + (long)t * N * D, w.dZout + (long)t * N * D, w.dXZ,
                                     w.DZ + (long)t * N * D, dhc, HCW, w.dU, w.dwf_part, att_fused ? nullptr : w.DA, d.B, d.R, d.L, D, A,
                                     use_b ? w.DHCb : nullptr, annb));
        if (use_b) {
            SAT_TRY(gemm_bb_nn(st, w.DHCb, HCW, w.Wcat_b, n, w.dHc, n, N, n, HCW, 1, slab, se));
        } else if (NL == 1) {
            SAT_TRY(gemm(st, A_ROW, B_KMAJOR, dhc, HCW, w.Wcat, n, w.dHc, n, N, n, HCW, 1, EPI_NONE, nullptr, nullptr, nullptr, nullptr, 0, 0, 0, slab, se));
        } else {
            SAT_TRY(gemm(st, A_ROW, B_KMAJOR, dhc, HCW, w.Wcat, n, dHcs(top), n, N, n, A + D, 1, EPI_NONE, nullptr, nullptr, nullptr, nullptr, 0, 0, 0, slab, se));
            SAT_TRY(gemm(st, A_ROW, B_KMAJOR, dhc + A + D, HCW, w.Wcat + (long)(A + D) * n, n, dHcs(0), n, N, n, 4 * n, 1, EPI_NONE, nullptr, nullptr, nullptr, nullptr, 0, 0, 0, slab, se));
        }
    }

    auto wgrad = [&](const float* dy, long ldy, const float* x, long ldx, float* out, long ldo, int M, int Nn) {
        return gemm(st, A_KMAJOR, B_KMAJOR, dy, ldy, x, ldx, out, ldo, M, Nn, KR, 0, EPI_NONE, nullptr, nullptr, nullptr, nullptr, 0, 0, 0, slab, se);
    };
    const float* dG = w.DHC + A + D;
    SAT_TRY(wgrad(w.DHC, HCW, Hs(0, top), n, g.att_dec, n, A, n));
    SAT_TRY(wgrad(w.DHC + A, HCW, Hs(0, top), n, g.beta_w, n, D, n));
    SAT_TRY(wgrad(dG, HCW, Hs(0, 0), n, g.w_hh, n, 4 * n, n));
    for (int l = 1; l < NL; ++l) {
        const float* dgu = DGUs(0, l);
        SAT_TRY(wgrad(dgu, 4 * n, Hs(1, l - 1), n, g.up_w_ih[l - 1], n, 4 * n, n));
        SAT_TRY(wgrad(dgu, 4 * n, Hs(0, l), n, g.up_w_hh[l - 1], n, 4 * n, n));
        SAT_TRY(colsum(st, w, dgu, 4 * n, KR, 4 * n, g.up_b_ih[l - 1]));
        SAT_TRY(dev_copy_bytes(st, g.up_b_hh[l - 1], g.up_b_ih[l - 1], (size_t)4 * n * 4));
    }
    SAT_TRY(colsum(st, w, w.DHC + A, HCW, KR, D, g.beta_b));
    SAT_TRY(colsum(st, w, dG, HCW, KR, 4 * n, g.b_ih));
    SAT_TRY(dev_copy_bytes(st, g.b_hh, g.b_ih, (size_t)4 * n * 4));
    SAT_TRY(wgrad(dG, HCW, w.Y, m, g.w_ih, m + D, 4 * n, m));
    SAT_TRY(wgrad(dG, HCW, w.XZ, D, g.w_ih + m, m + D, 4 * n, D));
    SAT_TRY(gemm(st, A_ROW, B_KMAJOR, dG, HCW, p.w_ih, m + D, w.dY, m, KR, m, 4 * n, 1));
    if (d.embedding_dropout > 0.f && KR > 0) {
        hipLaunchKernelGGL(dropout_rows_kernel, dim3(cdiv((long)KR * m, 256)), dim3(256), 0, st, w.dY, w.dY, (long)KR * m, m, d.embedding_dropout,
                           (unsigned long long)d.dropout_seed, 1u, 0L);
        SAT_TRY(launch_ok("embedding dropout bwd"));
    }
    if (KR > 0) {
        SAT_TRY(dev_fill_bytes(st, w.emb_count, 0, (size_t)V * 4));
        hipLaunchKernelGGL(embedding_count_kernel, dim3(cdiv(KR, 256)), dim3(256), 0, st, w.Tok, KR, V, d.padding_idx, w.emb_count);
        hipLaunchKernelGGL(embedding_scan_kernel, dim3(1), dim3(1024), 0, st, w.emb_count, V, w.emb_offset, w.emb_cursor);
        hipLaunchKernelGGL(embedding_place_kernel, dim3(cdiv(KR, 256)), dim3(256), 0, st, w.Tok, KR, V, d.padding_idx, w.emb_offset, w.emb_cursor, w.emb_list);
        hipLaunchKernelGGL(embedding_sum_kernel, dim3(V), dim3(256), 0, st, w.dY, w.Tok, w.emb_offset, w.emb_list, g.embedding, KR, m, d.padding_idx);
        SAT_TRY(launch_ok("embedding gradient"));
    } else SAT_TRY(dev_fill_bytes(st, g.embedding, 0, (size_t)V * m * 4));
    SAT_TRY(colsum(st, w, w.dwf_part, A, d.B, A, g.att_f));
    SAT_TRY(gemm(st, A_KMAJOR, B_KMAJOR, w.dU, A, b.ann, D, g.att_enc, D, A, D, d.B * d.L, 0, EPI_NONE, nullptr, nullptr, nullptr, nullptr, 0, 0, 0, slab, se));
    SAT_TRY(gemm(st, A_ROW, B_KMAJOR, w.dU, A, p.att_enc, D, dann, D, d.B * d.L, D, A));
    SAT_TRY(attention_context_bwd(alphas, w.DZ, b.lengths, dann, 1, d.B, d.R, T1, d.L, D, st));
    if (d.dropout > 0.f) {
        const int n2 = 2 * n * NL;
        SAT_TRY(dev_copy_bytes(st, w.init_rows, w.dHc, (size_t)NL * N * n * 4));
        SAT_TRY(dev_copy_bytes(st, w.init_rows + (long)NL * N * n, w.dCc, (size_t)NL * N * n * 4));
        SAT_TRY(gemm(st, A_KMAJOR, B_KMAJOR, w.init_rows, n2, w.f_rows, m, g.init_i_w, m, n2, m, N));
        SAT_TRY(colsum(st, w, w.init_rows, n2, N, n2, g.init_i_b));
        SAT_TRY(gemm(st, A_ROW, B_KMAJOR, w.init_rows, n2, p.init_i_w, m, w.df_rows, m, N, m, n2));
        SAT_TRY(gemm(st, A_KMAJOR, B_KMAJOR, w.df_rows, m, w.mean_rows, D, g.init_f_w, D, m, D, N));
        SAT_TRY(colsum(st, w, w.df_rows, m, N, m, g.init_f_b));
        SAT_TRY(gemm(st, A_ROW, B_KMAJOR, w.df_rows, m, p.init_f_w, D, w.mean_rows, D, N, D, m));
        hipLaunchKernelGGL(init_mean_rows_bwd_kernel, dim3(cdiv((long)d.B * D, 256)), dim3(256), 0, st, w.mean_rows, w.dmean, d.B, d.R, D, d.dropout,
                           (unsigned long long)d.dropout_seed);
        SAT_TRY(launch_ok("init_mean_rows_bwd"));
    } else {
    const int n2 = 2 * n * NL;
    hipLaunchKernelGGL(init_expand_bwd_kernel, dim3(cdiv((long)d.B * n2, 256)), dim3(256), 0, st, w.dHc, w.dCc, w.dinit_img, d.B, d.R, n * NL);
    SAT_TRY(launch_ok("init_expand_bwd"));
    SAT_TRY(gemm(st, A_KMAJOR, B_KMAJOR, w.dinit_img, n2, w.f, m, g.init_i_w, m, n2, m, d.B));
    SAT_TRY(colsum(st, w, w.dinit_img, n2, d.B, n2, g.init_i_b));
    SAT_TRY(gemm(st, A_ROW, B_KMAJOR, w.dinit_img, n2, p.init_i_w, m, w.df, m, d.B, m, n2));
    SAT_TRY(gemm(st, A_KMAJOR, B_KMAJOR, w.df, m, w.mean, D, g.init_f_w, D, m, D, d.B));
    SAT_TRY(colsum(st, w, w.df, m, d.B, m, g.init_f_b));
    SAT_TRY(gemm(st, A_ROW, B_KMAJOR, w.df, m, p.init_f_w, D, w.dmean, D, d.B, D, m));
    }
    const long tot = (long)d.B * d.L * D;
    hipLaunchKernelGGL(dann_add_mean_kernel, dim3(cdiv(tot, 256)), dim3(256), 0, st, dann, w.dmean, d.L, D, tot);
    return launch_ok("dann_add_mean");
}


int colsum_public(const float* x, long ld, long rows, int cols, float* out, float* scratch, hipStream_t st) {
    Ws w; w.colpart = scratch;
    return colsum(st, w, x, ld, (int)rows, cols, out);
}

size_t decoder_workspace_bytes(const sat_decoder_dims& d) { return layout(d, nullptr).total; }

struct InferWs { size_t total; float *U, *Wcat, *bcat, *mean, *f, *init_img, *hc, *Z, *XZ, *Y, *u, *gu, *bup, *sc; int* ones; };
static InferWs infer_layout(const sat_decoder_dims& d, int Kmax, char* base) {
    InferWs w; size_t off = 0;
    const long HCW = d.A + d.D + 4L * d.n;
    auto take = [&](size_t elems) { size_t o = off; off += (elems * 4 + 255) & ~(size_t)255; return base ? base + o : (char*)nullptr; };
    w.U = (float*)take((size_t)d.L * d.A); w.Wcat = (float*)take((size_t)HCW * d.n); w.bcat = (float*)take((size_t)HCW);
    w.mean = (float*)take(d.D); w.f = (float*)take(d.m); w.init_img = (float*)take(2 * (size_t)d.n * d.layers);
    w.gu = (float*)take((size_t)Kmax * 4 * d.n); w.bup = (float*)take((size_t)d.layers * 4 * d.n);
    w.hc = (float*)take((size_t)Kmax * HCW); w.Z = (float*)take((size_t)Kmax * d.D); w.XZ = (float*)take((size_t)Kmax * d.D);
    w.Y = (float*)take((size_t)Kmax * d.m); w.u = (float*)take((size_t)Kmax * d.m); w.ones = (int*)take(Kmax); w.sc = (float*)take((size_t)Kmax * d.L);
    w.total = off;
    return w;
}
size_t decoder_infer_workspace_bytes(const sat_decoder_dims& d, int Kmax) { return infer_layout(d, Kmax, nullptr).total; }

int decoder_infer_begin(const sat_decoder_dims& d, const sat_decoder_params& p, const float* ann, int K, int Kmax, float* h, float* c,
                        char* ws, size_t ws_bytes, hipStream_t st) {
    InferWs w = infer_layout(d, Kmax, ws);
    SAT_REQUIRE(ws_bytes >= w.total && K >= 1 && K <= Kmax, "decoder_infer_begin: workspace %zu < %zu or bad beam count %d/%d", ws_bytes, w.total, K, Kmax);
    t_bf16_mfma = d.precision ? 1 : 0;
    const int n = d.n, A = d.A, D = d.D, m = d.m;
    SAT_TRY(dev_copy_bytes(st, w.Wcat, p.att_dec, (size_t)A * n * 4));
    SAT_TRY(dev_copy_bytes(st, w.Wcat + (long)A * n, p.beta_w, (size_t)D * n * 4));
    SAT_TRY(dev_copy_bytes(st, w.Wcat + (long)(A + D) * n, p.w_hh, (size_t)4 * n * n * 4));
    SAT_TRY(dev_fill_bytes(st, w.bcat, 0, (size_t)A * 4));
    SAT_TRY(dev_copy_bytes(st, w.bcat + A, p.beta_b, (size_t)D * 4));
    hipLaunchKernelGGL(add_kernel, dim3(cdiv(4 * n, 256)), dim3(256), 0, st, w.bcat + A + D, p.b_ih, p.b_hh, (long)4 * n);
    SAT_TRY(launch_ok("bias add"));
// ... 460 lines not shown
```

### show-attend-and-tell-pytorch-lightning_amd/csrc/decoder_kernels.h

```cpp
#pragma once
#include "common.h"

namespace sat {

constexpr int ATT_RMAX = 8;
constexpr int ATT_THREADS = 256;

__global__ void fill_kernel(float* p, long n, float v) {
    long i = (long)blockIdx.x * blockDim.x + threadIdx.x;
    if (i < n) p[i] = v;
}

__global__ void cast_bf16_kernel(const float* __restrict__ src, __bf16* __restrict__ dst, long n4) {
    long e = (long)blockIdx.x * blockDim.x + threadIdx.x;
    if (e >= n4) return;
    const float4 v = reinterpret_cast<const float4*>(src)[e];
    typedef __bf16 b4 __attribute__((ext_vector_type(4)));
    b4 o; o[0] = (__bf16)v.x; o[1] = (__bf16)v.y; o[2] = (__bf16)v.z; o[3] = (__bf16)v.w;
    reinterpret_cast<b4*>(dst)[e] = o;
}

__global__ void cast_block_bf16_kernel(const float* __restrict__ src, long ld, __bf16* __restrict__ dst, int rows, int cols) {
    long e = (long)blockIdx.x * blockDim.x + threadIdx.x;
    const int c4 = cols / 4;
// ... 769 lines not shown
#pragma unroll
            for (int u = 0; u < U; ++u) {
                const int v = v0 + 256 * u;
                if (v >= V4) continue;
                const float e[4] = {q[u].x, q[u].y, q[u].z, q[u].w};
                float m4 = fmaxf(fmaxf(e[0], e[1]), fmaxf(e[2], e[3]));
#pragma unroll
                for (int i = 0; i < 4; ++i) {
                    tot += e[i];
                    if (e[i] > bv) { bv = e[i]; bi = 4 * v + i; }
                }
                if (m4 > mx) { sum *= __expf(mx - m4); mx = m4; }
                if (mx != -INFINITY) sum += (__expf(e[0] - mx) + __expf(e[1] - mx)) + (__expf(e[2] - mx) + __expf(e[3] - mx));
            }
        }
    } else {
        for (int v = tid; v < V; v += 256) {
            float xv = x[v];
            tot += xv;
            if (xv > bv || (xv == bv && v < bi)) { bv = xv; bi = v; }
            if (xv > mx) { sum = sum * __expf(mx - xv) + 1.f; mx = xv; } else sum += __expf(xv - mx);
        }
    }
    for (int o = 32; o > 0; o >>= 1) {
        float om = __shfl_xor(mx, o, 64), os = __shfl_xor(sum, o, 64);
        float nm = fmaxf(mx, om);
        float fa = (mx == nm) ? 1.f : __expf(mx - nm), fb = (om == nm) ? 1.f : __expf(om - nm);
        sum = sum * fa + os * fb; mx = nm;
        tot += __shfl_xor(tot, o, 64);
        float ob = __shfl_xor(bv, o, 64); int oi = __shfl_xor(bi, o, 64);
        if (ob > bv || (ob == bv && oi < bi)) { bv = ob; bi = oi; }
    }
    const int w = tid >> 6;
    if ((tid & 63) == 0) { s_m[w] = mx; s_s[w] = sum; s_t[w] = tot; s_b[w] = bv; s_i[w] = bi; }
    __syncthreads();
    if (tid == 0) {
        float M = fmaxf(fmaxf(s_m[0], s_m[1]), fmaxf(s_m[2], s_m[3]));
        float S = 0.f, Tt = 0.f, Bv = -INFINITY; int Bi = 0x7fffffff;
        for (int k = 0; k < 4; ++k) {
            S += (s_m[k] == M) ? s_s[k] : s_s[k] * __expf(s_m[k] - M); Tt += s_t[k];
            if (s_b[k] > Bv || (s_b[k] == Bv && s_i[k] < Bi)) { Bv = s_b[k]; Bi = s_i[k]; }
        }
        const float lse = M + __logf(S);
        const int t = target[p];
        float nll = lse - x[t];
        float smooth = lse - Tt / (float)V;
        lse_rows[p] = lse;
        loss_rows[p] = (1.f - smoothing) * nll + smoothing * smooth;
        correct_rows[p] = (Bi == t) ? 1 : 0;
    }
}
template <int VEC>
__global__ __launch_bounds__(256) void ce_grad_kernel(const float* __restrict__ logits, const int* __restrict__ target, const float* __restrict__ lse_rows,
                                                      int V, float smoothing, float inv_rows, const float* __restrict__ gscale, float* __restrict__ dlogits) {
    const int p = blockIdx.x;
    const float* x = logits + (long)p * V; float* g = dlogits + (long)p * V;
    const float lse = lse_rows[p], sv = smoothing / (float)V, conf = 1.f - smoothing;
    const float sc = inv_rows * (gscale ? gscale[0] : 1.f);
    const int t = target[p];
    if (VEC == 4) {
        constexpr int U = 4;
        const int V4 = V >> 2;
        for (int v0 = threadIdx.x; v0 < V4; v0 += 256 * U) {
            float4 q[U];
#pragma unroll
            for (int u = 0; u < U; ++u) { const int v = v0 + 256 * u; if (v < V4) q[u] = reinterpret_cast<const float4*>(x)[v]; }
#pragma unroll
            for (int u = 0; u < U; ++u) {
                const int v = v0 + 256 * u;
                if (v >= V4) continue;
                float4 o;
                o.x = (__expf(q[u].x - lse) - sv - ((4 * v == t) ? conf : 0.f)) * sc;
                o.y = (__expf(q[u].y - lse) - sv - ((4 * v + 1 == t) ? conf : 0.f)) * sc;
                o.z = (__expf(q[u].z - lse) - sv - ((4 * v + 2 == t) ? conf : 0.f)) * sc;
                o.w = (__expf(q[u].w - lse) - sv - ((4 * v + 3 == t) ? conf : 0.f)) * sc;
                reinterpret_cast<float4*>(g)[v] = o;
            }
        }
    } else {
        for (int v = threadIdx.x; v < V; v += 256) g[v] = (__expf(x[v] - lse) - sv - ((v == t) ? conf : 0.f)) * sc;
    }
}

__global__ void ce_finish_kernel(const float* __restrict__ loss_rows, const int* __restrict__ correct_rows, int P, float* __restrict__ out) {
    __shared__ double s_l[256]; __shared__ int s_c[256];
    double s = 0.0; int c = 0;
    for (int p = threadIdx.x; p < P; p += 256) { s += (double)loss_rows[p]; c += correct_rows[p]; }
    s_l[threadIdx.x] = s; s_c[threadIdx.x] = c;
    __syncthreads();
    for (int o = 128; o > 0; o >>= 1) { if ((int)threadIdx.x < o) { s_l[threadIdx.x] += s_l[threadIdx.x + o]; s_c[threadIdx.x] += s_c[threadIdx.x + o]; } __syncthreads(); }
    if (threadIdx.x == 0) { out[0] = (float)(s_l[0] / (double)P); out[1] = (float)s_c[0] / (float)P; }
}

__global__ void ds_rows_kernel(const float* __restrict__ alphas, float* __restrict__ asum, float* __restrict__ part, int N, int T1, int L) {
    __shared__ float s_p[256];
    long e = (long)blockIdx.x * 256 + threadIdx.x;
    float v = 0.f;
    if (e < (long)N * L) {
        long i = e / L; int l = (int)(e % L);
        float s = 0.f;
        for (int t = 0; t < T1; ++t) s += alphas[(i * T1 + t) * L + l];
        asum[e] = s;
        v = (1.f - s) * (1.f - s);
    }
    s_p[threadIdx.x] = v;
    __syncthreads();
    for (int o = 128; o > 0; o >>= 1) { if ((int)threadIdx.x < o) s_p[threadIdx.x] += s_p[threadIdx.x + o]; __syncthreads(); }
    if (threadIdx.x == 0) part[blockIdx.x] = s_p[0];
}
__global__ void ds_finish_kernel(const float* __restrict__ part, int nparts, float gamma, long count, float* __restrict__ out) {
    __shared__ double s_p[256];
    double s = 0.0;
    for (int p = threadIdx.x; p < nparts; p += 256) s += (double)part[p];
    s_p[threadIdx.x] = s;
    __syncthreads();
    for (int o = 128; o > 0; o >>= 1) { if ((int)threadIdx.x < o) s_p[threadIdx.x] += s_p[threadIdx.x + o]; __syncthreads(); }
    if (threadIdx.x == 0) out[0] = gamma * (float)(s_p[0] / (double)count);
}
__global__ void ds_grad_kernel(const float* __restrict__ asum, const float* __restrict__ gscale, float gamma, float* __restrict__ dalphas, int N, int T1, int L) {
    long e = (long)blockIdx.x * blockDim.x + threadIdx.x;
    if (e >= (long)N * T1 * L) return;
    long i = e / ((long)T1 * L); int l = (int)(e % L);
    float g = gscale ? gscale[0] : 1.f;
    dalphas[e] = g * gamma * 2.f * (asum[i * L + l] - 1.f) / (float)((long)N * L);
}

__global__ void colsum_part_kernel(const float* __restrict__ x, long ld, int rows, int cols, int rows_per, float* __restrict__ part) {
    int c = blockIdx.x * blockDim.x + threadIdx.x;
    if (c >= cols) return;
    int r0 = blockIdx.y * rows_per, r1 = min(rows, r0 + rows_per);
    float s = 0.f;
    for (int r = r0; r < r1; ++r) s += x[(long)r * ld + c];
    part[(long)blockIdx.y * cols + c] = s;
}
__global__ void colsum_part4_kernel(const float* __restrict__ x, long ld, int rows, int cols4, int rows_per, float* __restrict__ part) {
    const int c4 = blockIdx.x * blockDim.x + threadIdx.x;
    if (c4 >= cols4) return;
    const int r0 = blockIdx.y * rows_per, r1 = min(rows, r0 + rows_per);
    float4 a[4];
#pragma unroll
    for (int u = 0; u < 4; ++u) a[u] = make_float4(0.f, 0.f, 0.f, 0.f);
    int r = r0;
    for (; r + 3 < r1; r += 4) {
#pragma unroll
        for (int u = 0; u < 4; ++u) {
            const float4 v = *reinterpret_cast<const float4*>(x + (long)(r + u) * ld + 4 * c4);
            a[u].x += v.x; a[u].y += v.y; a[u].z += v.z; a[u].w += v.w;
        }
    }
    for (; r < r1; ++r) { const float4 v = *reinterpret_cast<const float4*>(x + (long)r * ld + 4 * c4); a[0].x += v.x; a[0].y += v.y; a[0].z += v.z; a[0].w += v.w; }
    float4 s;
    s.x = (a[0].x + a[1].x) + (a[2].x + a[3].x); s.y = (a[0].y + a[1].y) + (a[2].y + a[3].y);
    s.z = (a[0].z + a[1].z) + (a[2].z + a[3].z); s.w = (a[0].w + a[1].w) + (a[2].w + a[3].w);
    *reinterpret_cast<float4*>(part + (long)blockIdx.y * cols4 * 4 + 4 * c4) = s;
}
__global__ void colsum_finish_kernel(const float* __restrict__ part, int nparts, int cols, float* __restrict__ out, int accumulate, float scale) {
    int c = blockIdx.x * blockDim.x + threadIdx.x;
    if (c >= cols) return;
    float s = 0.f;
    for (int p = 0; p < nparts; ++p) s += part[(long)p * cols + c];
    s *= scale;
    out[c] = accumulate ? out[c] + s : s;
}

constexpr int EMB_LIST = 1024;
__global__ void embedding_count_kernel(const int* __restrict__ tok, int rows, int V, int padding_idx, int* __restrict__ count) {
// ... 577 lines not shown
```

### show-attend-and-tell-pytorch-lightning_amd/decoder.py

```python
import collections
import ctypes as C

import numpy as np
import torch

from . import _lib as L


def _upload(t, dev):
    if dev.type != "cuda":
        return t.to(dev)
    return t.pin_memory().to(dev, non_blocking=True)


class PackPlan:

    def __init__(self, lengths, T, device):
        lens = torch.as_tensor(lengths, dtype=torch.int64, device="cpu").reshape(-1)
        self.N, self.T, self.T1 = lens.numel(), int(T), int(T) - 1
        if (lens < 0).any() or (lens > self.T1).any():
            raise ValueError("caption lengths must lie in [0, T-1]")
        _, order = torch.sort(lens, descending=True)
        self.sorted_indices = order
        order_np, lens_np = order.numpy(), lens.numpy()
# ... 61 lines not shown
    if not 1 <= int(layers) <= L.MAX_LSTM_LAYERS:
        raise ValueError("decoder_layers=%d: the library is built for 1..%d stacked LSTM layers" % (layers, L.MAX_LSTM_LAYERS))
    return L.DecoderDims(B=B, R=R, T=T, L=Lc, D=D, A=A, m=m, n=n, V=V, P=P, deep_output=int(bool(deep)), padding_idx=padding_idx,
                         precision=int(precision), layers=int(layers), embed_max_norm=float(embed_max_norm or 0.0), dropout=float(dropout),
                         embedding_dropout=float(embedding_dropout), dropout_seed=int(dropout_seed))


def _params_struct(tensors, layers=1):
    s = L.DecoderParams()
    for k in L.PARAM_FIELDS:
        t = tensors.get(k)
        setattr(s, k, None if t is None else t.data_ptr())
    for k in L.UP_FIELDS:
        arr = getattr(s, k)
        for l in range(1, layers):
            arr[l - 1] = tensors["%s_l%d" % (k[3:], l)].data_ptr()
    return s


def layers_of(n_params):
    extra = n_params - len(L.PARAM_FIELDS)
    if extra < 0 or extra % len(L.UP_FIELDS):
        raise ValueError("decoder parameter list has %d entries; expected 18 + 4 per stacked layer" % n_params)
    return 1 + extra // len(L.UP_FIELDS)


def _check_param(name, t, shape):
    if t is None:
        return
    if tuple(t.shape) != tuple(shape):
        raise ValueError("decoder parameter %s has shape %s, expected %s" % (name, tuple(t.shape), tuple(shape)))
    if t.dtype != torch.float32 or not t.is_contiguous():
        raise ValueError("decoder parameter %s must be contiguous fp32" % name)


class DecoderTrainFn(torch.autograd.Function):

    @staticmethod
    def forward(ctx, ann, caps_i32, plan, teacher, deep, padding_idx, R, precision, embed_max_norm, dropout, *params):
        lib = L.lib()
        L.require_gpu(ann, caps_i32, *[p for p in params if p is not None])
        layers = layers_of(len(params))
        names = L.param_names(layers)
        tens = dict(zip(names, params))
        ann = ann.contiguous()
        B, Lc, D = ann.shape
        V, m = tens["embedding"].shape
        n = tens["w_hh"].shape[1]
        A = tens["att_dec"].shape[0]
        N, T = caps_i32.shape
        if N != B * R or plan.N != N or plan.T != T:
            raise ValueError("caption batch (%d,%d) does not match B*R=%d / plan (%d,%d)" % (N, T, B * R, plan.N, plan.T))
        shapes = dict(embedding=(V, m), init_f_w=(m, D), init_f_b=(m,), init_i_w=(2 * n * layers, m), init_i_b=(2 * n * layers,), w_ih=(4 * n, m + D),
                      w_hh=(4 * n, n), b_ih=(4 * n,), b_hh=(4 * n,), att_enc=(A, D), att_dec=(A, n), att_f=(1, A), beta_w=(D, n),
                      beta_b=(D,), out_hidden=(m, n), out_context=(m, D), out_w=(V, m), out_b=(V,))
        for l in range(1, layers):
            shapes.update({"w_ih_l%d" % l: (4 * n, n), "w_hh_l%d" % l: (4 * n, n), "b_ih_l%d" % l: (4 * n,), "b_hh_l%d" % l: (4 * n,)})
        for k in names:
            _check_param(k, tens[k], shapes[k])
            if tens[k] is None and k not in ("out_context", "out_b"):
                raise ValueError("decoder parameter %s is missing" % k)
        dims = decoder_dims(B, R, T, Lc, D, A, m, n, V, plan.P, deep, padding_idx, precision, embed_max_norm, *dropout, layers=layers)
        ws_bytes = lib.sat_decoder_workspace_bytes(C.byref(dims))
        if ws_bytes == 0:
            raise L.SatHipError("sat_decoder_workspace_bytes: %s" % lib.sat_last_error().decode())
        ws = torch.empty(ws_bytes, dtype=torch.uint8, device=ann.device)
        logits = torch.empty(max(plan.P, 1), V, dtype=torch.float32, device=ann.device)[:plan.P]
        alphas = torch.empty(N, T - 1, Lc, dtype=torch.float32, device=ann.device)
        teacher = np.ascontiguousarray(teacher, np.int32)
        batch = L.DecoderBatch(ann=ann.data_ptr(), caps=caps_i32.data_ptr(), lengths=plan.lengths.data_ptr(), prow=plan.prow.data_ptr(),
                               src_row=plan.src_row.data_ptr(), step_offsets_host=plan.offsets_host.ctypes.data,
                               teacher_host=teacher.ctypes.data)
        w = _params_struct(tens, layers)
        L.check(lib.sat_decoder_train_fwd(C.byref(dims), C.byref(w), C.byref(batch), L.ptr(logits), L.ptr(alphas), L.ptr(ws), ws_bytes,
                                          L.stream_ptr()), "sat_decoder_train_fwd")
        ctx.dims, ctx.plan, ctx.teacher, ctx.ws, ctx.ws_bytes = dims, plan, teacher, ws, ws_bytes
        ctx.caps, ctx.layers = caps_i32, layers
        ctx.save_for_backward(ann, alphas, *[p for p in params if p is not None])
        ctx.present = [p is not None for p in params]
        return logits, alphas

    @staticmethod
    def backward(ctx, dlogits, dalphas):
        lib = L.lib()
        saved = list(ctx.saved_tensors)
        ann, alphas = saved[0], saved[1]
        it = iter(saved[2:])
        params = [next(it) if present else None for present in ctx.present]
        names = L.param_names(ctx.layers)
        tens = dict(zip(names, params))
        plan, dims = ctx.plan, ctx.dims
        taken = set()

        def gbuf(t):
            if id(t) in taken:
                return torch.empty_like(t)
            taken.add(id(t))
            return L.grad_buffer(t)

        grads = {k: (None if t is None else gbuf(t)) for k, t in tens.items()}
        dann = torch.empty_like(ann)
        if dlogits is None:
            dlogits = torch.zeros(plan.P, dims.V, dtype=torch.float32, device=ann.device)
        dlogits = dlogits.contiguous()
        dalphas = None if dalphas is None else dalphas.contiguous()
        batch = L.DecoderBatch(ann=ann.data_ptr(), caps=ctx.caps.data_ptr(), lengths=plan.lengths.data_ptr(), prow=plan.prow.data_ptr(),
                               src_row=plan.src_row.data_ptr(), step_offsets_host=plan.offsets_host.ctypes.data,
                               teacher_host=ctx.teacher.ctypes.data)
        w, g = _params_struct(tens, ctx.layers), _params_struct(grads, ctx.layers)
        L.check(lib.sat_decoder_train_bwd(C.byref(dims), C.byref(w), C.byref(batch), L.ptr(dlogits), L.ptr(alphas), L.ptr(dalphas),
                                          C.byref(g), L.ptr(dann), L.ptr(ctx.ws), ctx.ws_bytes, L.stream_ptr()), "sat_decoder_train_bwd")
        return (dann, None, None, None, None, None, None, None, None, None, *[grads[k] for k in names])


class LabelSmoothingFn(torch.autograd.Function):

    @staticmethod
    def forward(ctx, logits, targets_i32, smoothing):
        lib = L.lib()
        L.require_gpu(logits, targets_i32)
        logits = logits.contiguous()
        P, V = logits.shape
        lse = torch.empty(P, dtype=torch.float32, device=logits.device)
        rows = torch.empty(P, dtype=torch.float32, device=logits.device)
        correct = torch.empty(P, dtype=torch.int32, device=logits.device)
        out = torch.empty(2, dtype=torch.float32, device=logits.device)
        L.check(lib.sat_ce_label_smooth_fwd(L.ptr(logits), L.ptr(targets_i32), P, V, float(smoothing), L.ptr(lse), L.ptr(rows),
                                            L.ptr(correct), L.ptr(out), L.stream_ptr()), "sat_ce_label_smooth_fwd")
        ctx.save_for_backward(logits, targets_i32, lse)
        ctx.smoothing = float(smoothing)
        loss, acc = out[0].clone(), out[1].clone()
        ctx.mark_non_differentiable(acc)
        return loss, acc

    @staticmethod
    def backward(ctx, gloss, _gacc):
        lib = L.lib()
        logits, targets, lse = ctx.saved_tensors
        P, V = logits.shape
        dlogits = torch.empty_like(logits)
        g = gloss.reshape(1).to(torch.float32).contiguous()
        L.check(lib.sat_ce_label_smooth_bwd(L.ptr(logits), L.ptr(targets), L.ptr(lse), P, V, ctx.smoothing, L.ptr(g), L.ptr(dlogits),
                                            L.stream_ptr()), "sat_ce_label_smooth_bwd")
        return dlogits, None, None


class DoublyStochasticFn(torch.autograd.Function):

    @staticmethod
    def forward(ctx, alphas, gamma):
        lib = L.lib()
        L.require_gpu(alphas)
        alphas = alphas.contiguous()
        N, T1, Lc = alphas.shape
        asum = torch.empty(N, Lc, dtype=torch.float32, device=alphas.device)
        part = torch.empty((N * Lc + 255) // 256, dtype=torch.float32, device=alphas.device)
        out = torch.empty(1, dtype=torch.float32, device=alphas.device)
        L.check(lib.sat_doubly_stochastic_fwd(L.ptr(alphas), N, T1, Lc, float(gamma), L.ptr(asum), L.ptr(part), L.ptr(out),
                                              L.stream_ptr()), "sat_doubly_stochastic_fwd")
        ctx.save_for_backward(asum)
        ctx.shape, ctx.gamma = (N, T1, Lc), float(gamma)
        return out[0].clone()

    @staticmethod
    def backward(ctx, g):
        lib = L.lib()
        (asum,) = ctx.saved_tensors
        N, T1, Lc = ctx.shape
        dal = torch.empty(N, T1, Lc, dtype=torch.float32, device=asum.device)
        gs = g.reshape(1).to(torch.float32).contiguous()
        L.check(lib.sat_doubly_stochastic_bwd(L.ptr(asum), L.ptr(gs), N, T1, Lc, ctx.gamma, L.ptr(dal), L.stream_ptr()),
                "sat_doubly_stochastic_bwd")
        return dal, None


def dropout_scale_reference(seed, stream, idx, p):
    M = (1 << 64) - 1
    idx = np.asarray(idx, dtype=np.uint64)
    with np.errstate(over="ignore"):
        z = (np.uint64(seed & M) + np.uint64((0x9E3779B97F4A7C15 * (stream + 1)) & M) + idx * np.uint64(0xD1342543DE82EF95))
        z = (z ^ (z >> np.uint64(30))) * np.uint64(0xBF58476D1CE4E5B9)
        z = (z ^ (z >> np.uint64(27))) * np.uint64(0x94D049BB133111EB)
        z ^= z >> np.uint64(31)
    u = (z >> np.uint64(40)).astype(np.float32) * np.float32(1.0 / 16777216.0)
    return np.where(u >= np.float32(p), np.float32(1.0) / (np.float32(1.0) - np.float32(p)), np.float32(0.0)).astype(np.float32)


def gemm(A, B, *, amode=0, bmode=0, M=None, N=None, K=None, out=None, accumulate=False, epi=0, bias=None, e0=None, c0=0, c1=0,
         a_rows=None, c_rows=None, out_rows=None, slab=None, bf16_mfma=False, out_dtype=torch.float32):
    lib = L.lib()
    L.require_gpu(A, B)
    if M is None:
        M = (a_rows.numel() if a_rows is not None else A.shape[0]) if amode == 0 else A.shape[1]
    if K is None:
        K = A.shape[1] if amode == 0 else A.shape[0]
    if N is None:
        N = B.shape[0] if bmode == 0 else B.shape[1]
    if out is None:
        out = torch.zeros(out_rows if out_rows is not None else M, N, dtype=out_dtype, device=A.device)
    d = L.GemmDesc(A=A.data_ptr(), lda=A.stride(0), a_rows=None if a_rows is None else a_rows.data_ptr(),
                   B=B.data_ptr(), ldb=B.stride(0), C=out.data_ptr(), ldc=out.stride(0),
                   c_rows=None if c_rows is None else c_rows.data_ptr(), M=M, N=N, K=K, amode=amode, bmode=bmode,
                   accumulate=int(accumulate), epi=epi, bias=None if bias is None else bias.data_ptr(),
                   e0=None if e0 is None else e0.data_ptr(), lde0=0 if e0 is None else e0.stride(0), c0=c0, c1=c1,
                   slab=None if slab is None else slab.data_ptr(), slab_elems=0 if slab is None else slab.numel())
    bf = torch.bfloat16
    if bf16_mfma or A.dtype == bf or B.dtype == bf or out.dtype == bf:
        t = L.GemmTypes(a_bf16=int(A.dtype == bf), b_bf16=int(B.dtype == bf), c_bf16=int(out.dtype == bf), bf16_mfma=int(bf16_mfma))
        L.check(lib.sat_gemm_ex(C.byref(d), C.byref(t), L.stream_ptr()), "sat_gemm_ex")
    else:
        L.check(lib.sat_gemm_f32(C.byref(d), L.stream_ptr()), "sat_gemm_f32")
    return out
```

### show-attend-and-tell-pytorch-lightning_amd/graph.py

```python
import collections

import numpy as np
import torch

from . import _lib as L
from . import decoder as Dk
from . import encoder as E


class _Ctx:

    def save_for_backward(self, *tensors):
        self.saved_tensors = tuple(tensors)

    def mark_non_differentiable(self, *tensors):
        pass


class _Entry:
    __slots__ = ("graph", "img", "caps", "lengths", "out", "grads", "keep", "opt_bufs", "opt_sig", "replays")


class GraphedTrainStep:
    def __init__(self, model, optimizer, sync=None, max_graphs=4, enabled=True):
        self.model, self.opt, self.sync = model, optimizer, sync
        self.enabled = bool(enabled)
        self.max_graphs = int(max_graphs)
        self._graphs = collections.OrderedDict()
        self._pool = None
        self._stream = None
        self._current = None
        self._params = [p for g in optimizer.param_groups for p in g["params"]]
        self.stats = collections.Counter()

    def _why_eager(self, img):
        import torch.distributed as dist
        hp = self.model.hp
        if not self.enabled:
            return "disabled"
        if not img.is_cuda:
            return "cpu batch"
        if dist.is_available() and dist.is_initialized() and dist.get_world_size() > 1:
            return "more than one process"
        if int(getattr(hp, "accumulate", 1) or 1) > 1:
            return "gradient accumulation"
        if self.model.training and (float(hp.dropout) > 0.0 or float(hp.embedding_dropout) > 0.0):
            return "dropout"
        if not hasattr(self.opt, "step_device"):
            return "optimizer is not a FusedOptimizer"
        return None

    def _params_sig(self):
        return tuple([(p.data_ptr(), p.requires_grad) for p in self._params])

    def _stale_copies(self):
        for p in self._params:
            if getattr(p, "_sat_bf16_shadow", None) is not None and p._sat_shadow_version != p._version:
                return True
        return False

    def _eager(self, batch, epsilon, gstep, teacher):
        self._current = None
        self.opt.zero_grad(set_to_none=True)
        loss = self.model._step_losses(batch, epsilon, teacher=teacher)
        acc = self.model.criterion.last_accuracy
        self.model._step_end(gstep)
        loss.backward()
        if self.sync is not None:
            self.sync.finish()
        self.opt.step()
        return {"loss": loss.detach(), "accuracy": acc, "epsilon_tf": float(epsilon)}

    def _capture_stream(self, dev):
        if self._stream is None:
            self._stream = torch.cuda.Stream(dev)
            self._pool = torch.cuda.graph_pool_handle()
        return self._stream

    def _eager_on_capture_stream(self, batch, epsilon, gstep, teacher):
        cur = torch.cuda.current_stream(batch[0].device)
        side = self._capture_stream(batch[0].device)
        side.wait_stream(cur)
        with torch.cuda.stream(side):
            out = self._eager(batch, epsilon, gstep, teacher)
        cur.wait_stream(side)
        for t in (batch[0], batch[1]):
            t.record_stream(side)
        return out

    def _forward_backward(self, batch, epsilon, teacher):
        model = self.model
        img, caps, lengths = batch
        hp = model.hp
        enc = model.encoder
        with torch.no_grad():
            enc_params = list(enc.parameters())
            ectx = _Ctx()
            try:
                ann = enc.Fn._forward(ectx, img, enc, *enc_params)
            finally:
                E._defer[0] = False
            Bn, D, h, w = ann.shape
            ann_bld = ann.permute(0, 2, 3, 1).reshape(Bn, h * w, D)
            _, R, T = caps.shape
            plan = Dk.PackPlan.cached(lengths.reshape(-1), T, img.device)
            caps2 = caps.reshape(Bn * R, T)
            caps_i32 = caps2.to(dtype=torch.int32).contiguous()
            dec_params = model.param_list()
            dctx = _Ctx()
            logits, alphas = Dk.DecoderTrainFn.forward(dctx, ann_bld, caps_i32, plan, teacher, bool(hp.deep_output), model.pad_idx, R,
                                                       int(model.sat_precision == "bf16"), getattr(hp, "embed_norm", None) or 0.0,
                                                       model._dropout_args(None), *dec_params)
            targets = plan.pack(caps2[:, 1:].unsqueeze(-1)).squeeze(-1)
            cctx, sctx = _Ctx(), _Ctx()
            ce, acc = Dk.LabelSmoothingFn.forward(cctx, logits, targets.to(torch.int32), model.criterion.smoothing)
            model.criterion.last_accuracy = acc
            ds = Dk.DoublyStochasticFn.forward(sctx, alphas, float(hp.att_gamma))
            loss = ce + ds
            one = torch.ones((), dtype=torch.float32, device=img.device)
            dlogits = Dk.LabelSmoothingFn.backward(cctx, one, None)[0]
            dalphas = Dk.DoublyStochasticFn.backward(sctx, one)[0]
            douts = Dk.DecoderTrainFn.backward(dctx, dlogits, dalphas)
            dann = douts[0]
            grads = {}

            def give(p, g):
                if p is None or g is None or not p.requires_grad:
                    return
                if id(p) in grads:
                    grads[id(p)][1].add_(g)
                else:
                    grads[id(p)] = (p, g)

            for p, g in zip(dec_params, douts[10:]):
                give(p, g)
            if any(p.requires_grad for p in enc_params):
                eouts = enc.Fn.backward(ectx, dann.reshape(Bn, h, w, D).permute(0, 3, 1, 2))
                for p, g in zip(enc_params, eouts[2:]):
                    give(p, g)
            for p, g in grads.values():
                p.grad = g
        return loss, acc

    def _capture(self, key, batch, epsilon, teacher):
        img, caps, lengths = batch
        dev = img.device
        ent = _Entry()
        ent.img, ent.caps, ent.lengths = img.clone(), caps.clone(), lengths
        self._capture_stream(dev)
        self.opt.zero_grad(set_to_none=True)
        self.opt.prepare_device_step(dev)
        torch.cuda.synchronize(dev)
        g = torch.cuda.CUDAGraph()
        with torch.cuda.graph(g, pool=self._pool, stream=self._stream):
            out_loss, acc = self._forward_backward((ent.img, ent.caps, ent.lengths), epsilon, teacher)
            if self.sync is not None:
                self.sync.finish()
            self.opt.step_device()
        ent.graph = g
        ent.out = {"loss": out_loss, "accuracy": acc, "epsilon_tf": float(epsilon)}
        ent.grads = [(p, p.grad) for p in self._params if p.grad is not None]
        ent.keep = [list(E._slabs.values()), list(E._bn_scratch_buf.values()), Dk.PackPlan.cached(lengths.reshape(-1), caps.shape[-1], dev), teacher]
        ent.opt_bufs = self.opt.device_buffers()
        ent.opt_sig = self.opt.table_signature()
        ent.replays = 0
        self._graphs[key] = ent
        while len(self._graphs) > self.max_graphs:
            self._graphs.popitem(last=False)
        self.stats["captured"] += 1
        return ent

    def __call__(self, batch, batch_idx=0):
        model = self.model
        img, caps, lengths = batch
        lengths = torch.as_tensor(lengths).cpu()
        batch = (img, caps, lengths)
        epsilon, gstep = model._step_begin()
        plan = Dk.PackPlan.cached(lengths.reshape(-1), caps.shape[-1], img.device)
        teacher = plan.teacher_flags(float(epsilon))
        why = self._why_eager(img)
        if why is not None:
            self.stats["eager: " + why] += 1
            return self._eager(batch, epsilon, gstep, teacher)
        key = (tuple(img.shape), tuple(caps.shape), lengths.numpy().tobytes(), np.asarray(teacher, np.int32).tobytes(), float(epsilon),
               model.sat_precision, model.training, self._params_sig())
        stale = self._stale_copies()
        if stale:
            self._graphs.clear()
        if key not in self._graphs:
            self._graphs[key] = None
            self.stats["eager: first step of a shape / plan"] += 1
            return self._eager_on_capture_stream(batch, epsilon, gstep, teacher)
        ent = self._graphs[key]
        self._graphs.move_to_end(key)
        if ent is None:
            ent = self._capture(key, batch, epsilon, teacher)
        else:
            if img.data_ptr() != ent.img.data_ptr():
                ent.img.copy_(img, non_blocking=True)
            if caps.data_ptr() != ent.caps.data_ptr():
                ent.caps.copy_(caps, non_blocking=True)
        if self._current is not ent:
            for p, gr in ent.grads:
                p.grad = gr
            self._current = ent
# ... 11 lines not shown
```

### show-attend-and-tell-pytorch-lightning_amd/model.py

```python
import math
from types import SimpleNamespace

import torch
import torch.nn.functional as F
from torch import nn

from torch.nn.utils.rnn import PackedSequence
from torch.optim.lr_scheduler import MultiStepLR, ReduceLROnPlateau, ExponentialLR, CosineAnnealingWarmRestarts, OneCycleLR

from . import _lib as L
from . import constraints
from . import decoder as Dk
from .modules import DeepOutput, Embedding, Gate, InitLSTM, LSTM, SoftAttention
from .encoder import get_encoder

try:
    import pytorch_lightning as pl
    _Base = pl.LightningModule
except Exception:
    pl = None
    _Base = nn.Module


class _HParams(dict):
# ... 340 lines not shown
                with torch.cuda.graph(g):
                    enqueue(ann_s, o)
                while len(cache) >= 4:
                    cache.pop(next(iter(cache)))
                ent = cache[key] = (g, ann_s, o, _keep)
            g, ann_s, o = ent[0], ent[1], ent[2]
            ann_s.copy_(ann_bld)
            g.replay()
        else:
            o = buffers()
            enqueue(ann_bld, o)
        return o

    @torch.no_grad()
    def beam_decode_batched(self, ann_bld, hw, beamk=3, max_gen_length=32, temperature=1.0, rescore_method=None, rescore_reward=0.5,
                            return_all=False, sample_method="beam", sample_topk=3, decoder_noise=None, seed=None, gumbel=None, normals=None, graph=False,
                            topg=None, prefix=None, banned=None, no_unk=False, sample_topp=0.9):
        import numpy as np
        o = self._beam_search_device(ann_bld, beamk, max_gen_length, temperature, sample_method, sample_topk, decoder_noise, seed, gumbel, normals, graph,
                                     topg, prefix, banned, no_unk, sample_topp)
        B = ann_bld.shape[0]
        Hh, Ww = hw
        K, S = int(beamk), int(max_gen_length)
        tok_in, prev_row, alpha_hist = o["tok_in"], o["prev_row"], o["alpha_hist"]
        fin_count, fin_step, fin_row, fin_score, fin_mean = o["fin_count"], o["fin_step"], o["fin_row"], o["fin_score"], o["fin_mean"]
        tok_in, prev_row = tok_in.cpu().numpy(), prev_row.cpu().numpy()
        alpha_np = alpha_hist.cpu().numpy()
        fin_count, fin_step, fin_row = fin_count.cpu().numpy(), fin_step.cpu().numpy(), fin_row.cpu().numpy()
        fin_score, fin_mean = fin_score.cpu(), fin_mean.cpu()
        bidx = np.repeat(np.arange(B), K)[(np.arange(K)[None, :] < fin_count[:, None]).reshape(-1)]
        fidx = np.tile(np.arange(K), B)[(np.arange(K)[None, :] < fin_count[:, None]).reshape(-1)]
        hstep, cur = fin_step[bidx, fidx].astype(np.int64), fin_row[bidx, fidx].astype(np.int64)
        nh = len(bidx)
        rows = np.zeros((S + 1, nh), np.int64)
        for s_ in range(S, -1, -1):
            act = hstep >= s_
            rows[s_, act] = cur[act]
            if s_ > 0:
                cur[act] = prev_row[s_, bidx[act], cur[act]]
        sidx = np.arange(S + 1)[:, None]
        toks_all = tok_in[sidx, bidx[None, :], rows]
        als_all = torch.from_numpy(alpha_np[sidx, bidx[None, :], rows])
        if rescore_method == "LN":
            resc = fin_score[bidx, fidx] / torch.from_numpy(hstep).float()
        elif rescore_method == "WR":
            resc = fin_score[bidx, fidx] + rescore_reward * torch.from_numpy(hstep).float()
        elif rescore_method == "BAR":
            resc = fin_score[bidx, fidx] + rescore_reward * (-fin_mean[bidx, fidx])
        else:
            resc = fin_score[bidx, fidx]
        ppl_all = torch.exp(-fin_score[bidx, fidx] / torch.from_numpy(hstep).float())
        resc, ppl_all = resc.tolist(), ppl_all.tolist()
        captions, cap_scores, cap_alphas, cap_ppl = [], [], [], []
        hpos = 0
        for b in range(B):
            fin_caps, fin_alphas, fin_scores, fin_ppl = [], [], [], []
            for f in range(int(fin_count[b])):
                hh, step = hpos + f, int(hstep[hpos + f])
                fin_caps.append(toks_all[1:step + 1, hh].tolist())
                fin_alphas.append(als_all[:step, hh].reshape(-1, Hh, Ww).clone())
                fin_scores.append(resc[hh]); fin_ppl.append(ppl_all[hh])
            hpos += int(fin_count[b])
            if return_all:
                order = [i for _, i in sorted([[fin_scores[i], i] for i in range(len(fin_scores))], reverse=True)]
                captions.append([fin_caps[i] for i in order]); cap_alphas.append([fin_alphas[i] for i in order])
                cap_scores.append([fin_scores[i] for i in order]); cap_ppl.append([fin_ppl[i] for i in order])
            else:
                best = fin_scores.index(max(fin_scores))
                captions.append(fin_caps[best]); cap_alphas.append(fin_alphas[best])
                cap_scores.append(fin_scores[best]); cap_ppl.append(fin_ppl[best])
        return captions, cap_scores, cap_alphas, cap_ppl

    def _dropout_args(self, seed=None):
        p, pe = float(self.hp.dropout), float(self.hp.embedding_dropout)
        if not self.training or (p == 0.0 and pe == 0.0):
            return (0.0, 0.0, 0)
        if seed is None:
            gen = self.__dict__.get("_dropout_gen")
            if gen is None:
                gen = self.__dict__["_dropout_gen"] = torch.Generator().manual_seed(torch.initial_seed() & 0x7FFFFFFFFFFFFFFF)
            seed = int(torch.randint(0, 2 ** 62, (1,), generator=gen))
        return (p, pe, int(seed))

    def train_decode(self, ann_bld, caps, lengths, epsilon=0, draw=None, with_loss=True, dropout_seed=None, teacher=None):
        B, R, T = caps.shape
        plan = Dk.PackPlan.cached(lengths.reshape(-1).cpu(), T, ann_bld.device)
        if teacher is None:
            teacher = plan.teacher_flags(float(epsilon), draw)
        caps2 = caps.reshape(B * R, T)
        caps_i32 = caps2.to(device=ann_bld.device, dtype=torch.int32).contiguous()
        logits_packed, alphas = Dk.DecoderTrainFn.apply(ann_bld, caps_i32, plan, teacher, bool(self.hp.deep_output), self.pad_idx, R,
                                                        int(getattr(self, "sat_precision", "fp32") == "bf16"), getattr(self.hp, "embed_norm", None) or 0.0,
                                                        self._dropout_args(dropout_seed), *self.param_list())
        targets_packed = plan.pack(caps2[:, 1:].to(ann_bld.device).unsqueeze(-1)).squeeze(-1)
        if not with_loss:
            return dict(logits_packed=logits_packed, targets_packed=targets_packed, alphas=alphas, plan=plan)
        ce = self.criterion(logits_packed, targets_packed)
        ds = Dk.DoublyStochasticFn.apply(alphas, float(self.hp.att_gamma))
        return dict(logits_packed=logits_packed, targets_packed=targets_packed, alphas=alphas, ce=ce, ds=ds,
                    acc=self.criterion.last_accuracy, plan=plan)


class SAT(SATDecoder, _Base):

    def __init__(self, **kwargs):
        nn.Module.__init__(self)
        hp = _HParams(kwargs)
        for k, v in dict(encoder_size=None, embed_norm=None, pretrained_embedding=None, pretrained=False, decoder_tf=None,
                         decoder_tf_min=0.5, epochs=10, encoder_finetune_after=-1, att_gamma=1.0, label_smoothing=0.0,
                         dropout=0.0, embedding_dropout=0.0, weight_tying=False, deep_output=False, decoder_layers=1,
                         lr_warmup_steps=0).items():
            hp.setdefault(k, v)
        self.scheduler = None
        self.opt_init_lr = None
        self.__dict__["_sat_global_step"] = 0
        self.__dict__["_sat_micro_batches"] = 0
        self._build_decoder(hp, encoder_factory=get_encoder)
        amp = str(hp.get("precision", 32)) in ("16", "bf16", "16-mixed", "bf16-mixed")
        self.set_precision(hp.get("hip_precision", "bf16" if amp else "fp32"))
        if hp.pretrained_embedding is not None:
            import numpy as np
            self.embedding.weight = nn.Parameter(torch.tensor(np.load(hp.pretrained_embedding), dtype=torch.float32))
        self.special_idxs = [self.stoi("<PAD>"), self.stoi("<START>"), self.stoi("<END>")]

    def set_precision(self, mode):
        if mode not in ("fp32", "bf16"):
            raise ValueError("hip_precision must be 'fp32' or 'bf16'")
        self.sat_precision = mode
        self.encoder.precision = mode

    @property
    def hparams(self):
        return self.hp

    def stoi(self, s):
        return int(self.hp.vocab_stoi.get(s, self.hp.vocab_stoi["<UNK>"]))

    def itos(self, i):
        return str(self.hp.vocab_itos.get(int(i), "<UNK>"))

    def decode_seq(self, seq, remove_special=False):
        return [str(self.itos(t)) for t in seq if not (remove_special and t in self.special_idxs)]

    def encode(self, img):
        ann = self.encoder(img)
        B, D, h, w = ann.shape
        return ann.permute(0, 2, 3, 1).reshape(B, h * w, D), (h, w)

    @torch.no_grad()
    def caption(self, img_tensor, beamk=3, max_gen_length=32, temperature=1.0, sample_method="beam", sample_topk=3,
                decoder_noise=None, rescore_method=None, rescore_reward=0.5, return_all=False, topg=None, prefix=None, banned=None, no_unk=False,
                sample_topp=0.9):
        self.eval()
        return self.forward(img_tensor, beamk, max_gen_length, temperature, sample_method, sample_topk, decoder_noise,
                            rescore_method, rescore_reward, return_all, topg, prefix, banned, no_unk, sample_topp)

    def forward(self, img, beamk=3, max_gen_length=32, temperature=1.0, sample_method="beam", sample_topk=3, decoder_noise=None,
                rescore_method=None, rescore_reward=0.5, return_all=False, topg=None, prefix=None, banned=None, no_unk=False, sample_topp=0.9):
        assert sample_method in SAMPLE_METHODS
        check_sample_topp(sample_method, sample_topp)
        con = dict(topg=topg, prefix=prefix, banned=banned, no_unk=no_unk)
        constraints.resolve(self.hp.vocab_stoi, self.hp.vocab_size, img.shape[0], beamk, max_gen_length, sample_method, **con)
        with torch.no_grad():
            ann_bld, hw = self.encode(img)
            if max_gen_length >= 1:
                return self.beam_decode_batched(ann_bld.contiguous(), hw, beamk, max_gen_length, temperature, rescore_method, rescore_reward, return_all,
                                                sample_method=sample_method, sample_topk=sample_topk, decoder_noise=decoder_noise,
                                                graph=bool(self.__dict__.get("beam_graph", False)), sample_topp=sample_topp, **con)
            return self.beam_decode(ann_bld.contiguous(), hw, beamk, max_gen_length, temperature, sample_method, sample_topk,
                                    decoder_noise, rescore_method, rescore_reward, return_all, sample_topp=sample_topp, **con)

    def train_batch(self, batch, epsilon=0, draw=None, teacher=None):
        img, encoded_captions, lengths = batch
        ann_bld, _ = self.encode(img)
        res = self.train_decode(ann_bld, encoded_captions, lengths, float(epsilon), draw, with_loss=False, teacher=teacher)
        plan = res["plan"]
        lp = PackedSequence(res["logits_packed"], plan.batch_sizes, plan.sorted_indices_dev, plan.unsorted_indices_dev)
        tp = PackedSequence(res["targets_packed"], plan.batch_sizes, plan.sorted_indices_dev, plan.unsorted_indices_dev)
        return lp, tp, res["alphas"]

    def calibrate_temperature(self, batches, max_batches=42, **fit_kwargs):
        from . import calibration
        return calibration.calibrate_temperature(self, batches, max_batches, **fit_kwargs)

    def teacher_forcing_epsilon(self, current_epoch=0):
        hp = self.hp
        if hp.decoder_tf is None:
            return 0.0
        if hp.decoder_tf == "always":
            return 1.0
        if hp.decoder_tf == "linear":
            return 1 - (1 - hp.decoder_tf_min) * current_epoch / hp.epochs
        if hp.decoder_tf == "inv_sigmoid":
            l = -math.log(hp.decoder_tf_min / (1 - hp.decoder_tf_min)); g = 5.0
            b = (1 / ((l / g) + 1)) * hp.epochs
            return 1 / (1 + math.exp((g / b) * (current_epoch - b)))
        if hp.decoder_tf == "exp":
            return math.exp(math.log(hp.decoder_tf_min) / hp.epochs) ** current_epoch
        raise ValueError("decoder_tf=%r" % (hp.decoder_tf,))

    def sat_global_step(self):
        tr = getattr(self, "_trainer", None) if pl is not None else None
        if tr is not None:
            return int(tr.global_step)
        return int(self.__dict__["_sat_global_step"])

    def _train_optimizer(self):
        if pl is not None and getattr(self, "_trainer", None) is not None:
            return self.optimizers()
        return self.__dict__.get("_sat_optimizer")

    def step_learning_rate(self, gstep):
        hp = self.hp
        opt = self._train_optimizer()
        if opt is None or self.opt_init_lr is None:
            return
        if gstep < hp.lr_warmup_steps:
            lr_scale = min(1, float(gstep + 1) / hp.lr_warmup_steps)
            for pg, init_lr in zip(opt.param_groups, self.opt_init_lr):
                pg["lr"] = lr_scale * init_lr
        elif gstep > 0:
            if type(self.scheduler) in [CosineAnnealingWarmRestarts, OneCycleLR]:
                self.scheduler.step()

    def _step_begin(self):
        hp = self.hp
        epoch = int(getattr(self, "current_epoch", 0) or 0)
        epsilon = self.teacher_forcing_epsilon(epoch)
        gstep = self.sat_global_step()
        if gstep == hp.encoder_finetune_after and hp.encoder_finetune_after >= 0:
            for p in self.encoder.parameters():
                p.requires_grad = True
        return epsilon, gstep

    def _step_losses(self, batch, epsilon, teacher=None):
        lp, tp, alphas = self.train_batch(batch, epsilon, teacher=teacher)
        loss = self.criterion(lp.data, tp.data)
        loss = loss + Dk.DoublyStochasticFn.apply(alphas, float(self.hp.att_gamma))
        return loss

    def _step_end(self, gstep):
        hp = self.hp
        self.step_learning_rate(gstep)
        micro = self.__dict__["_sat_micro_batches"] + 1
        if micro >= max(1, int(getattr(hp, "accumulate", 1) or 1)):
            self.__dict__["_sat_global_step"] += 1
            micro = 0
        self.__dict__["_sat_micro_batches"] = micro

    def training_step(self, batch, batch_idx=0):
        epsilon, gstep = self._step_begin()
        loss = self._step_losses(batch, epsilon)
        self._step_end(gstep)
        return {"loss": loss, "accuracy": self.criterion.last_accuracy, "epsilon_tf": float(epsilon)}

    def _log_scalar(self, key, val, step):
        logger = getattr(self, "logger", None)
        exp = getattr(logger, "experiment", None)
        if exp is not None and hasattr(exp, "add_scalar"):
            exp.add_scalar(key, val, global_step=step)

    def training_epoch_end(self, outputs):
        epoch = int(getattr(self, "current_epoch", 0))
        means = {}
        for k in outputs[0].keys():
            vals = [float(x[k]) for x in outputs]
            means[k] = sum(vals) / len(vals) if vals else 0
            self._log_scalar("{}/train_epoch".format(k), means[k], epoch + 1)
        if isinstance(getattr(self, "scheduler", None), (MultiStepLR, ExponentialLR)):
            self.scheduler.step()
        return means

    @torch.no_grad()
    def score_captions(self, captions, encoded_captions, lengths, perplexities=None):
        from . import metrics
        lens = lengths.tolist() if torch.is_tensor(lengths) else lengths
        references = [[c[1:l] for c, l in zip(refs, lens[i])] for i, refs in enumerate(encoded_captions.tolist())]
        out = {"bleu1": metrics.corpus_bleu(references, captions, weights=(1, 0, 0, 0)),
               "bleu2": metrics.corpus_bleu(references, captions, weights=(0.5, 0.5, 0, 0)),
               "bleu3": metrics.corpus_bleu(references, captions, weights=(0.33, 0.33, 0.33, 0)),
               "bleu4": metrics.corpus_bleu(references, captions, weights=(0.25, 0.25, 0.25, 0.25))}
        dev = self.embedding.weight.device
        enc = encoded_captions.to(dev)
        E = self.embedding.weight
        cossims = torch.zeros(enc.shape[0], dtype=torch.float, device=dev)
        for i in range(enc.shape[0]):
            cv = E[torch.as_tensor(captions[i], dtype=torch.long, device=dev)].mean(0).unsqueeze(0)
            rvs = torch.zeros(enc.shape[1], dtype=torch.float, device=dev)
            for j, l in enumerate(lens[i]):
                rv = E[enc[i][j][1:l]].mean(0).unsqueeze(0)
                rvs[j] = F.cosine_similarity(rv, cv)
            cossims[i] = rvs.max()
        out["cosine_similarity"] = cossims.mean().item()
        out["gleu"] = metrics.corpus_gleu(references, captions)
        if type(perplexities) == list:
            out["perplexity"] = sum(perplexities) / len(perplexities)
        return out

    def val_batch(self, batch, beamk=3, max_gen_length=32, temperature=0.5, sample_method="beam", sample_topk=3, decoder_noise=None,
                  rescore_method=None, rescore_reward=0.5, topg=None, prefix=None, banned=None, no_unk=False, sample_topp=0.9):
        img, encoded_captions, lengths = batch
        captions, scores, alphas, perplexities = self.caption(img, beamk, max_gen_length, temperature, sample_method, sample_topk, decoder_noise,
                                                              rescore_method, rescore_reward, return_all=False, topg=topg, prefix=prefix, banned=banned,
                                                              no_unk=no_unk, sample_topp=sample_topp)
        return self.score_captions(captions, encoded_captions, lengths, perplexities)

    def caption_tokens(self, img, beamk=3, max_gen_length=32, temperature=1.0, sample_method="beam", sample_topk=3, decoder_noise=None,
                       rescore_method=None, rescore_reward=0.5, seed=None, graph=False, topg=None, prefix=None, banned=None, no_unk=False, sample_topp=0.9):
        from . import evaluation
        return evaluation.caption_tokens(self, img, beamk, max_gen_length, temperature, sample_method, sample_topk, decoder_noise, rescore_method,
                                         rescore_reward, seed, graph, topg, prefix, banned, no_unk, sample_topp)

    def val_batch_stats(self, batch, beamk=3, max_gen_length=32, temperature=0.5, sample_method="beam", sample_topk=3, decoder_noise=None,
                        rescore_method=None, rescore_reward=0.5, seed=None, graph=False, corpus=None, topg=None, prefix=None, banned=None, no_unk=False,
                        sample_topp=0.9, chrf=None, chrf_beta=3.0):
        from . import evaluation
        return evaluation.val_batch_stats(self, batch, beamk, max_gen_length, temperature, sample_method, sample_topk, decoder_noise, rescore_method,
                                          rescore_reward, seed, graph, corpus, topg, prefix, banned, no_unk, sample_topp, chrf, chrf_beta)
# ... 93 lines not shown
```

Baseline: 32140 captions/s.

## Fuse label-smoothing CE backward into decoder backward with bf16 logit gradients

Adds a fused decoder+loss autograd path for bf16 mode. The cross-entropy backward now writes the logit gradient straight to bf16 and folds the output-bias column sum into that kernel. The output-projection data and weight gradients then run as bf16 MFMA GEMMs instead of fp32 GEMMs over a large P×V fp32 dlogits buffer. It also keeps per-timestep bf16 XZ/DHC buffers, so later backward steps can reuse them, at the cost of more workspace and bf16 rounding of the logit gradient.

```diff
diff --git a/include/sat_hip.h b/include/sat_hip.h
--- a/include/sat_hip.h
+++ b/include/sat_hip.h
@@ -99,10 +99,18 @@
                           const float* dlogits_packed, const float* alphas , const float* dalphas,
                           const sat_decoder_params* g, float* dann, void* workspace, size_t workspace_bytes, void* stream);
 
+int sat_decoder_loss_handoff(const sat_decoder_dims* d);
+int sat_decoder_train_bwd_ce(const sat_decoder_dims* d, const sat_decoder_params* w, const sat_decoder_batch* b,
+                             const float* logits_packed, const int32_t* targets, const float* lse_rows, float smoothing,
+                             const float* gscale, void* dlogits_bf16, const float* alphas, const float* dalphas,
+                             const sat_decoder_params* g, float* dann, void* workspace, size_t workspace_bytes, void* stream);
+
 int sat_ce_label_smooth_fwd(const float* logits, const int32_t* targets, int32_t P, int32_t V, float smoothing,
                             float* lse_rows, float* loss_rows, int32_t* correct_rows, float* out, void* stream);
 int sat_ce_label_smooth_bwd(const float* logits, const int32_t* targets, const float* lse_rows, int32_t P, int32_t V,
                             float smoothing, const float* gscale, float* dlogits, void* stream);
+int sat_ce_label_smooth_bwd_bf16(const float* logits, const int32_t* targets, const float* lse_rows, int32_t P, int32_t V,
+                                 float smoothing, const float* gscale, void* dlogits_bf16, float* dbias, float* scratch, void* stream);
 int sat_doubly_stochastic_fwd(const float* alphas, int32_t N, int32_t T1, int32_t L, float gamma,
                               float* asum, float* part, float* out, void* stream);
 int sat_doubly_stochastic_bwd(const float* asum, const float* gscale, int32_t N, int32_t T1, int32_t L, float gamma,
diff --git a/show-attend-and-tell-pytorch-lightning_amd/_lib.py b/show-attend-and-tell-pytorch-lightning_amd/_lib.py
--- a/show-attend-and-tell-pytorch-lightning_amd/_lib.py
+++ b/show-attend-and-tell-pytorch-lightning_amd/_lib.py
@@ -136,6 +136,12 @@
     "sat_decoder_train_bwd": (C.c_int, [C.POINTER(DecoderDims), C.POINTER(DecoderParams), C.POINTER(DecoderBatch),
                                         C.c_void_p, C.c_void_p, C.c_void_p, C.POINTER(DecoderParams), C.c_void_p,
                                         C.c_void_p, C.c_size_t, C.c_void_p]),
+    "sat_decoder_loss_handoff": (C.c_int, [C.POINTER(DecoderDims)]),
+    "sat_decoder_train_bwd_ce": (C.c_int, [C.POINTER(DecoderDims), C.POINTER(DecoderParams), C.POINTER(DecoderBatch),
+                                           C.c_void_p, C.c_void_p, C.c_void_p, C.c_float, C.c_void_p, C.c_void_p, C.c_void_p, C.c_void_p,
+                                           C.POINTER(DecoderParams), C.c_void_p, C.c_void_p, C.c_size_t, C.c_void_p]),
+    "sat_ce_label_smooth_bwd_bf16": (C.c_int, [C.c_void_p, C.c_void_p, C.c_void_p, C.c_int32, C.c_int32, C.c_float, C.c_void_p,
+                                               C.c_void_p, C.c_void_p, C.c_void_p, C.c_void_p]),
     "sat_ce_label_smooth_fwd": (C.c_int, [C.c_void_p, C.c_void_p, C.c_int32, C.c_int32, C.c_float, C.c_void_p, C.c_void_p,
                                           C.c_void_p, C.c_void_p, C.c_void_p]),
     "sat_ce_label_smooth_bwd": (C.c_int, [C.c_void_p, C.c_void_p, C.c_void_p, C.c_int32, C.c_int32, C.c_float, C.c_void_p,
diff --git a/show-attend-and-tell-pytorch-lightning_amd/csrc/api.hip b/show-attend-and-tell-pytorch-lightning_amd/csrc/api.hip
--- a/show-attend-and-tell-pytorch-lightning_amd/csrc/api.hip
+++ b/show-attend-and-tell-pytorch-lightning_amd/csrc/api.hip
@@ -44,6 +44,7 @@
     if (!strcmp(name, "glds_tall_k")) { glds_tall_k() = value; return SAT_OK; }
     if (!strcmp(name, "glds_tall_conv")) { glds_tall_conv() = value; return SAT_OK; }
     if (!strcmp(name, "tile_override")) { gemm_tile_override() = value; return SAT_OK; }
+    if (!strcmp(name, "bf16_handoff")) { bf16_handoff_switch() = value ? 1 : 0; return SAT_OK; }
     return fail(SAT_EINVAL, "debug_option: unknown option %s", name);
 }
 const char* sat_last_error(void) { return last_error_buf(); }
@@ -103,6 +104,27 @@
     return decoder_bwd(*d, *w, *b, dlogits_packed, alphas, dalphas, *g, dann, (char*)workspace, workspace_bytes, (hipStream_t)stream);
 }
 
+int sat_decoder_loss_handoff(const sat_decoder_dims* d) {
+    if (check_dims(d) != SAT_OK) return 0;
+    return decoder_bf16_handoff(*d);
+}
+int sat_decoder_train_bwd_ce(const sat_decoder_dims* d, const sat_decoder_params* w, const sat_decoder_batch* b, const float* logits_packed,
+                             const int32_t* targets, const float* lse_rows, float smoothing, const float* gscale, void* dlogits_bf16,
+                             const float* alphas, const float* dalphas, const sat_decoder_params* g, float* dann, void* workspace,
+                             size_t workspace_bytes, void* stream) {
+    SAT_TRY(check_dims(d)); SAT_TRY(check_params(d, w, "decoder_train_bwd_ce")); SAT_TRY(check_params(d, g, "decoder_train_bwd_ce(grads)")); SAT_TRY(check_batch(b));
+    if (!alphas || !dann || !workspace || !logits_packed || !targets || !lse_rows || !dlogits_bf16) return fail(SAT_EINVAL, "decoder_train_bwd_ce: null input/output/workspace");
+    if (!decoder_bf16_handoff(*d)) return fail(SAT_EUNSUPPORTED, "decoder_train_bwd_ce: these dimensions keep the fp32 gradient (sat_decoder_loss_handoff() == 0)");
+    if (!(smoothing >= 0.f && smoothing < 1.f)) return fail(SAT_EINVAL, "decoder_train_bwd_ce: smoothing %g out of range", smoothing);
+    const CeHandoff ce = {logits_packed, targets, lse_rows, smoothing, gscale, dlogits_bf16};
+    return decoder_bwd(*d, *w, *b, nullptr, alphas, dalphas, *g, dann, (char*)workspace, workspace_bytes, (hipStream_t)stream, &ce);
+}
+
+int sat_ce_label_smooth_bwd_bf16(const float* logits, const int32_t* targets, const float* lse_rows, int32_t P, int32_t V, float smoothing,
+                                 const float* gscale, void* dlogits_bf16, float* dbias, float* scratch, void* stream) {
+    if (!logits || !targets || !lse_rows || !dlogits_bf16 || (dbias && !scratch)) return fail(SAT_EINVAL, "ce_label_smooth_bwd_bf16: null pointer");
+    return ce_bwd_bf16(logits, targets, lse_rows, P, V, smoothing, gscale, dlogits_bf16, dbias, scratch, (hipStream_t)stream);
+}
 int sat_ce_label_smooth_fwd(const float* logits, const int32_t* targets, int32_t P, int32_t V, float smoothing, float* lse_rows,
                             float* loss_rows, int32_t* correct_rows, float* out, void* stream) {
     if (!logits || !targets || !lse_rows || !loss_rows || !correct_rows || !out) return fail(SAT_EINVAL, "ce_label_smooth_fwd: null pointer");
diff --git a/show-attend-and-tell-pytorch-lightning_amd/csrc/decoder.h b/show-attend-and-tell-pytorch-lightning_amd/csrc/decoder.h
--- a/show-attend-and-tell-pytorch-lightning_amd/csrc/decoder.h
+++ b/show-attend-and-tell-pytorch-lightning_amd/csrc/decoder.h
@@ -8,8 +8,14 @@
 size_t decoder_workspace_bytes(const sat_decoder_dims& d);
 int decoder_fwd(const sat_decoder_dims& d, const sat_decoder_params& p, const sat_decoder_batch& b, float* logits, float* alphas,
                 char* ws, size_t ws_bytes, hipStream_t st);
+struct CeHandoff { const float* logits; const int* targets; const float* lse_rows; float smoothing; const float* gscale; void* dlogits_bf16; };
 int decoder_bwd(const sat_decoder_dims& d, const sat_decoder_params& p, const sat_decoder_batch& b, const float* dlogits,
-                const float* alphas, const float* dalphas, const sat_decoder_params& g, float* dann, char* ws, size_t ws_bytes, hipStream_t st);
+                const float* alphas, const float* dalphas, const sat_decoder_params& g, float* dann, char* ws, size_t ws_bytes, hipStream_t st,
+                const CeHandoff* ce = nullptr);
+int decoder_bf16_handoff(const sat_decoder_dims& d);
+int& bf16_handoff_switch();
+int ce_bwd_bf16(const float* logits, const int* targets, const float* lse_rows, int P, int V, float smoothing, const float* gscale, void* dlogits_bf16,
+                float* dbias, float* scratch, hipStream_t st);
 enum { ATT_OP_FWD = 0, ATT_OP_BWD = 1, ATT_OP_CONTEXT_BWD = 2 };
 enum { ATT_FORM_SPLIT = 0, ATT_FORM_SINGLE = 1 };
 enum : unsigned { ATT_HAS_SCRATCH = 1, ATT_ANN_ALIGNED = 2, ATT_ROWS_ALIGNED = 4, ATT_HAS_BF16 = 8 };
diff --git a/show-attend-and-tell-pytorch-lightning_amd/csrc/decoder.hip b/show-attend-and-tell-pytorch-lightning_amd/csrc/decoder.hip
--- a/show-attend-and-tell-pytorch-lightning_amd/csrc/decoder.hip
+++ b/show-attend-and-tell-pytorch-lightning_amd/csrc/decoder.hip
@@ -60,9 +60,9 @@
     w.Hb = w.XZb = w.Wcat_b = w.Wz_b = w.DHCb = nullptr;
     w.annb = (d.precision && d.D % 4 == 0 && d.A % 4 == 0) ? (__bf16*)take((size_t)d.B * d.L * d.D, 2) : nullptr;
     if (d.precision && d.layers == 1 && d.n % 64 == 0 && d.D % 64 == 0 && d.A % 4 == 0 && d.m % 4 == 0) {
-        w.Hb = (__bf16*)take((size_t)(T1 + 1) * N * d.n, 2); w.XZb = (__bf16*)take((size_t)N * d.D, 2);
+        w.Hb = (__bf16*)take((size_t)(T1 + 1) * N * d.n, 2); w.XZb = (__bf16*)take((size_t)T1 * N * d.D, 2);
         w.Wcat_b = (__bf16*)take((size_t)HCW * d.n, 2); w.Wz_b = (__bf16*)take((size_t)4 * d.n * d.D, 2);
-        w.DHCb = (__bf16*)take((size_t)N * HCW, 2);
+        w.DHCb = (__bf16*)take((size_t)T1 * N * HCW, 2);
     }
     w.flags = (int*)take((size_t)d.V);
     w.emb_count = (int*)take((size_t)d.V); w.emb_offset = (int*)take((size_t)d.V + 1); w.emb_cursor = (int*)take((size_t)d.V);
@@ -127,10 +127,18 @@
     return launch_gemm(g, st);
 }
 
-static int gemm_bb_nn(hipStream_t st, const __bf16* A, long lda, const __bf16* B, long ldb, float* C, long ldc, int M, int N, int K, int acc, float* slab, long slab_elems) {
+static int gemm_bb_nn(hipStream_t st, const __bf16* A, long lda, const __bf16* B, long ldb, float* C, long ldc, int M, int N, int K, int acc, float* slab, long slab_elems,
+                      int epi = EPI_NONE, const float* e0 = nullptr, long lde0 = 0) {
     GemmArgs g;
     g.A = A; g.lda = lda; g.B = B; g.ldb = ldb; g.C = C; g.ldc = ldc; g.M = M; g.N = N; g.K = K;
     g.amode = A_ROW; g.bmode = B_KMAJOR; g.a_bf16 = g.b_bf16 = 1; g.c_bf16 = 0; g.bf16_mfma = 1; g.accumulate = acc; g.slab = slab; g.slab_elems = slab_elems;
+    g.epi = epi; g.e0 = e0; g.lde0 = lde0;
+    return launch_gemm(g, st);
+}
+static int gemm_bb_tn(hipStream_t st, const __bf16* A, long lda, const __bf16* B, long ldb, float* C, long ldc, int M, int N, int K, float* slab, long slab_elems) {
+    GemmArgs g;
+    g.A = A; g.lda = lda; g.B = B; g.ldb = ldb; g.C = C; g.ldc = ldc; g.M = M; g.N = N; g.K = K;
+    g.amode = A_KMAJOR; g.bmode = B_KMAJOR; g.a_bf16 = g.b_bf16 = 1; g.c_bf16 = 0; g.bf16_mfma = 1; g.slab = slab; g.slab_elems = slab_elems;
     return launch_gemm(g, st);
 }
 
@@ -462,8 +470,8 @@
             SAT_TRY(gemm(st, A_ROW, B_ROW, Hs(t, 0), n, w.Wcat + (long)(A + D) * n, n, hc + A + D, HCW, N, 4 * n, n, 0, EPI_BIAS, w.bcat + A + D));
         }
         SAT_TRY(launch_attention_fwd(st, b.ann, w.U, hc, HCW, p.att_f, b.lengths, t, alphas, T1, w.Z + (long)t * N * D, w.XZ + (long)t * N * D,
-                                     d.B, d.R, d.L, D, A, w.SC, use_b ? w.XZb : nullptr, annb));
-        if (use_b) SAT_TRY(gemm_bb_nt(st, w.XZb, D, w.Wz_b, D, hc + A + D, HCW, N, 4 * n, D, EPI_NONE, nullptr, 1));
+                                     d.B, d.R, d.L, D, A, w.SC, use_b ? w.XZb + (long)t * N * D : nullptr, annb));
+        if (use_b) SAT_TRY(gemm_bb_nt(st, w.XZb + (long)t * N * D, D, w.Wz_b, D, hc + A + D, HCW, N, 4 * n, D, EPI_NONE, nullptr, 1));
         else SAT_TRY(gemm(st, A_ROW, B_ROW, w.XZ + (long)t * N * D, D, p.w_ih + m, m + D, hc + A + D, HCW, N, 4 * n, D, 1));
         hipLaunchKernelGGL(lstm_cell_fwd_kernel, dim3(cdiv((long)N * n, 256)), dim3(256), 0, st, hc + A + D, HCW, w.GY + (long)t * N * 4 * n,
                            Cs(t, 0), Hs(t, 0), Cs(t + 1, 0), Hs(t + 1, 0), b.lengths, t, N, n, use_b ? w.Hb + (long)(t + 1) * N * n : (__bf16*)nullptr);
@@ -480,8 +488,28 @@
     return flush_outputs(st, d, p, b, w, logits, b.step_offsets_host[pending], b.step_offsets_host[ts]);
 }
 
+int& bf16_handoff_switch() { static int v = 1; return v; }
+int decoder_bf16_handoff(const sat_decoder_dims& d) {
+    return bf16_handoff_switch() && d.precision && d.layers == 1 && d.P > 0 && d.n % 64 == 0 && d.D % 64 == 0 && d.m % 64 == 0 && d.V % 8 == 0;
+}
+
+int ce_bwd_bf16(const float* logits, const int* targets, const float* lse_rows, int P, int V, float smoothing, const float* gscale, void* dlogits_bf16,
+                float* dbias, float* scratch, hipStream_t st) {
+    SAT_REQUIRE(P > 0 && V > 0, "ce_bwd_bf16: empty input");
+    SAT_REQUIRE(V % 4 == 0 && (uintptr_t)logits % 16 == 0 && (uintptr_t)dlogits_bf16 % 8 == 0, "ce_bwd_bf16: V=%d must be a multiple of 4 and the matrices aligned", V);
+    SAT_REQUIRE(!dbias || ((uintptr_t)scratch % 16 == 0 && scratch), "ce_bwd_bf16: the column sums need 16-byte aligned scratch");
+    const int nparts = cdiv(P, 256);
+    hipLaunchKernelGGL(ce_grad_bf16_kernel, dim3(cdiv(V / 4, 128), nparts), dim3(128), 0, st, logits, targets, lse_rows, P, V / 4, 256, smoothing, 1.0f / (float)P, gscale,
+                       reinterpret_cast<__bf16*>(dlogits_bf16), dbias ? scratch : (float*)nullptr);
+    SAT_TRY(launch_ok("ce_grad_bf16"));
+    if (!dbias) return SAT_OK;
+    hipLaunchKernelGGL(colsum_finish_kernel, dim3(cdiv(V, 256)), dim3(256), 0, st, scratch, nparts, V, dbias, 0, 1.f);
+    return launch_ok("colsum_finish");
+}
+
 int decoder_bwd(const sat_decoder_dims& d, const sat_decoder_params& p, const sat_decoder_batch& b, const float* dlogits,
-                       const float* alphas, const float* dalphas, const sat_decoder_params& g, float* dann, char* ws, size_t ws_bytes, hipStream_t st) {
+                       const float* alphas, const float* dalphas, const sat_decoder_params& g, float* dann, char* ws, size_t ws_bytes, hipStream_t st,
+                       const CeHandoff* ce) {
     Ws w = layout(d, ws);
     t_bf16_mfma = d.precision ? 1 : 0;
     SAT_REQUIRE(ws_bytes >= w.total, "decoder_bwd: workspace %zu < %zu bytes", ws_bytes, w.total);
@@ -501,16 +529,29 @@
     SAT_TRY(dev_fill_bytes(st, w.zero_begin, 0, (size_t)(w.zero_end - w.zero_begin)));
     if (NL > 1 && KR < T1 * N) SAT_TRY(dev_fill_bytes(st, w.DGU, 0, (size_t)(NL - 1) * T1 * N * 4 * n * 4));
 
+    const __bf16* dlb = nullptr;
     if (P > 0) {
-        SAT_TRY(gemm(st, A_ROW, B_KMAJOR, dlogits, V, p.out_w, m, w.dA, m, P, m, V, 0, d.deep_output ? EPI_MUL_DTANH : EPI_NONE, nullptr,
-                     nullptr, nullptr, w.Uact, m, 0, 0, slab, se));
+        const float* uin = d.dropout > 0.f ? w.Udrop : w.Uact;
+        if (ce) {
+            SAT_REQUIRE(decoder_bf16_handoff(d) && w.Wb_out && w.Ub, "decoder_bwd: the bf16 hand-off needs bf16 mode, one LSTM layer, n, D, m multiples of 64 and V of 8");
+            dlb = reinterpret_cast<const __bf16*>(ce->dlogits_bf16);
+            SAT_TRY(ce_bwd_bf16(ce->logits, ce->targets, ce->lse_rows, P, V, ce->smoothing, ce->gscale, ce->dlogits_bf16, g.out_b, w.colpart, st));
+            SAT_TRY(gemm_bb_nn(st, dlb, V, w.Wb_out, m, w.dA, m, P, m, V, 0, slab, se, d.deep_output ? EPI_MUL_DTANH : EPI_NONE, d.deep_output ? w.Uact : nullptr, m));
+        } else {
+            SAT_TRY(gemm(st, A_ROW, B_KMAJOR, dlogits, V, p.out_w, m, w.dA, m, P, m, V, 0, d.deep_output ? EPI_MUL_DTANH : EPI_NONE, nullptr,
+                         nullptr, nullptr, w.Uact, m, 0, 0, slab, se));
+        }
         if (d.dropout > 0.f) {
             hipLaunchKernelGGL(dropout_rows_kernel, dim3(cdiv((long)P * m, 256)), dim3(256), 0, st, w.dA, w.dA, (long)P * m, m, d.dropout,
                                (unsigned long long)d.dropout_seed, 2u, 0L);
             SAT_TRY(launch_ok("output dropout bwd"));
         }
-        SAT_TRY(gemm(st, A_KMAJOR, B_KMAJOR, dlogits, V, d.dropout > 0.f ? w.Udrop : w.Uact, m, g.out_w, m, V, m, P, 0, EPI_NONE, nullptr, nullptr, nullptr, nullptr, 0, 0, 0, slab, se));
-        if (g.out_b) SAT_TRY(colsum(st, w, dlogits, V, P, V, g.out_b));
+        if (ce) {
+            SAT_TRY(gemm_bb_tn(st, dlb, V, w.Ub, m, g.out_w, m, V, m, P, slab, se));
+        } else {
+            SAT_TRY(gemm(st, A_KMAJOR, B_KMAJOR, dlogits, V, uin, m, g.out_w, m, V, m, P, 0, EPI_NONE, nullptr, nullptr, nullptr, nullptr, 0, 0, 0, slab, se));
+            if (g.out_b) SAT_TRY(colsum(st, w, dlogits, V, P, V, g.out_b));
+        }
         SAT_TRY(gemm(st, A_ROW, B_KMAJOR, w.dA, m, p.out_hidden, n, w.dHout, n, P, n, m, 0, EPI_NONE, nullptr, nullptr, b.src_row));
         if (d.deep_output)
             SAT_TRY(gemm(st, A_ROW, B_KMAJOR, w.dA, m, p.out_context, D, w.dZout, D, P, D, m, 0, EPI_NONE, nullptr, nullptr, b.src_row));
@@ -533,6 +574,7 @@
     for (int t = ts - 1; t >= 0; --t) {
         const float* hc = w.HC + (long)t * N * HCW;
         float* dhc = w.DHC + (long)t * N * HCW;
+        __bf16* dhcb = use_b ? w.DHCb + (long)t * N * HCW : nullptr;
         for (int l = top; l >= 1; --l) {
             float* dgu = DGUs(t, l);
             hipLaunchKernelGGL(lstm_cell_bwd_kernel, dim3(cdiv((long)N * n, 256)), dim3(256), 0, st, GUs(t, l), 4 * n, Cs(t, l), Cs(t + 1, l),
@@ -543,15 +585,15 @@
         }
         hipLaunchKernelGGL(lstm_cell_bwd_kernel, dim3(cdiv((long)N * n, 256)), dim3(256), 0, st, hc + A + D, HCW, Cs(t, 0),
                            Cs(t + 1, 0), top == 0 ? w.dHout + (long)t * N * n : (const float*)nullptr, dHcs(0), dCcs(0), dhc + A + D, HCW, b.lengths, t, N, n,
-                           use_b ? w.DHCb + A + D : (__bf16*)nullptr);
+                           use_b ? dhcb + A + D : (__bf16*)nullptr);
         SAT_TRY(launch_ok("lstm_cell_bwd"));
-        if (use_b) SAT_TRY(gemm_bb_nn(st, w.DHCb + A + D, HCW, w.Wz_b, D, w.dXZ, D, N, D, 4 * n, 0, slab, se));
+        if (use_b) SAT_TRY(gemm_bb_nn(st, dhcb + A + D, HCW, w.Wz_b, D, w.dXZ, D, N, D, 4 * n, 0, slab, se));
         else SAT_TRY(gemm(st, A_ROW, B_KMAJOR, dhc + A + D, HCW, p.w_ih + m, m + D, w.dXZ, D, N, D, 4 * n, 0, EPI_NONE, nullptr, nullptr, nullptr, nullptr, 0, 0, 0, slab, se));
         SAT_TRY(launch_attention_bwd(st, b.ann, w.U, hc, HCW, p.att_f, b.lengths, t, alphas, dalphas, T1, w.Z + (long)t * N * D, w.dZout + (long)t * N * D, w.dXZ,
                                      w.DZ + (long)t * N * D, dhc, HCW, w.dU, w.dwf_part, att_fused ? nullptr : w.DA, d.B, d.R, d.L, D, A,
-                                     use_b ? w.DHCb : nullptr, annb));
+                                     dhcb, annb));
         if (use_b) {
-            SAT_TRY(gemm_bb_nn(st, w.DHCb, HCW, w.Wcat_b, n, w.dHc, n, N, n, HCW, 1, slab, se));
+            SAT_TRY(gemm_bb_nn(st, dhcb, HCW, w.Wcat_b, n, w.dHc, n, N, n, HCW, 1, slab, se));
         } else if (NL == 1) {
             SAT_TRY(gemm(st, A_ROW, B_KMAJOR, dhc, HCW, w.Wcat, n, w.dHc, n, N, n, HCW, 1, EPI_NONE, nullptr, nullptr, nullptr, nullptr, 0, 0, 0, slab, se));
         } else {
@@ -564,9 +606,17 @@
         return gemm(st, A_KMAJOR, B_KMAJOR, dy, ldy, x, ldx, out, ldo, M, Nn, KR, 0, EPI_NONE, nullptr, nullptr, nullptr, nullptr, 0, 0, 0, slab, se);
     };
     const float* dG = w.DHC + A + D;
-    SAT_TRY(wgrad(w.DHC, HCW, Hs(0, top), n, g.att_dec, n, A, n));
-    SAT_TRY(wgrad(w.DHC + A, HCW, Hs(0, top), n, g.beta_w, n, D, n));
-    SAT_TRY(wgrad(dG, HCW, Hs(0, 0), n, g.w_hh, n, 4 * n, n));
+    const bool wg_b = use_b && bf16_handoff_switch() && KR > 0 && A % 8 == 0;
+    const __bf16* dGb = w.DHCb + A + D;
+    if (wg_b) {
+        SAT_TRY(gemm_bb_tn(st, w.DHCb, HCW, w.Hb, n, g.att_dec, n, A, n, KR, slab, se));
+        SAT_TRY(gemm_bb_tn(st, w.DHCb + A, HCW, w.Hb, n, g.beta_w, n, D, n, KR, slab, se));
+        SAT_TRY(gemm_bb_tn(st, dGb, HCW, w.Hb, n, g.w_hh, n, 4 * n, n, KR, slab, se));
+    } else {
+        SAT_TRY(wgrad(w.DHC, HCW, Hs(0, top), n, g.att_dec, n, A, n));
+        SAT_TRY(wgrad(w.DHC + A, HCW, Hs(0, top), n, g.beta_w, n, D, n));
+        SAT_TRY(wgrad(dG, HCW, Hs(0, 0), n, g.w_hh, n, 4 * n, n));
+    }
     for (int l = 1; l < NL; ++l) {
         const float* dgu = DGUs(0, l);
         SAT_TRY(wgrad(dgu, 4 * n, Hs(1, l - 1), n, g.up_w_ih[l - 1], n, 4 * n, n));
@@ -578,7 +628,8 @@
     SAT_TRY(colsum(st, w, dG, HCW, KR, 4 * n, g.b_ih));
     SAT_TRY(dev_copy_bytes(st, g.b_hh, g.b_ih, (size_t)4 * n * 4));
     SAT_TRY(wgrad(dG, HCW, w.Y, m, g.w_ih, m + D, 4 * n, m));
-    SAT_TRY(wgrad(dG, HCW, w.XZ, D, g.w_ih + m, m + D, 4 * n, D));
+    if (wg_b) SAT_TRY(gemm_bb_tn(st, dGb, HCW, w.XZb, D, g.w_ih + m, m + D, 4 * n, D, KR, slab, se));
+    else SAT_TRY(wgrad(dG, HCW, w.XZ, D, g.w_ih + m, m + D, 4 * n, D));
     SAT_TRY(gemm(st, A_ROW, B_KMAJOR, dG, HCW, p.w_ih, m + D, w.dY, m, KR, m, 4 * n, 1));
     if (d.embedding_dropout > 0.f && KR > 0) {
         hipLaunchKernelGGL(dropout_rows_kernel, dim3(cdiv((long)KR * m, 256)), dim3(256), 0, st, w.dY, w.dY, (long)KR * m, m, d.embedding_dropout,
diff --git a/show-attend-and-tell-pytorch-lightning_amd/csrc/decoder_kernels.h b/show-attend-and-tell-pytorch-lightning_amd/csrc/decoder_kernels.h
--- a/show-attend-and-tell-pytorch-lightning_amd/csrc/decoder_kernels.h
+++ b/show-attend-and-tell-pytorch-lightning_amd/csrc/decoder_kernels.h
@@ -875,6 +875,47 @@
     }
 }
 
+__global__ __launch_bounds__(128) void ce_grad_bf16_kernel(const float* __restrict__ logits, const int* __restrict__ target, const float* __restrict__ lse_rows,
+                                                           int rows, int V4, int rows_per, float smoothing, float inv_rows, const float* __restrict__ gscale,
+                                                           __bf16* __restrict__ dlogits, float* __restrict__ part) {
+    typedef __bf16 b4 __attribute__((ext_vector_type(4)));
+    const int c4 = blockIdx.x * blockDim.x + threadIdx.x;
+    if (c4 >= V4) return;
+    const int V = 4 * V4;
+    const int r0 = blockIdx.y * rows_per, r1 = min(rows, r0 + rows_per);
+    const float sv = smoothing / (float)V, conf = 1.f - smoothing;
+    const float sc = inv_rows * (gscale ? gscale[0] : 1.f);
+    float4 a[4];
+#pragma unroll
+    for (int u = 0; u < 4; ++u) a[u] = make_float4(0.f, 0.f, 0.f, 0.f);
+    auto one = [&](int r, const float4& q, float4& acc) {
+#pragma clang fp contract(off)
+        const float lse = lse_rows[r]; const int t = target[r];
+        float4 o;
+        o.x = (__expf(q.x - lse) - sv - ((4 * c4 == t) ? conf : 0.f)) * sc;
+        o.y = (__expf(q.y - lse) - sv - ((4 * c4 + 1 == t) ? conf : 0.f)) * sc;
+        o.z = (__expf(q.z - lse) - sv - ((4 * c4 + 2 == t) ? conf : 0.f)) * sc;
+        o.w = (__expf(q.w - lse) - sv - ((4 * c4 + 3 == t) ? conf : 0.f)) * sc;
+        acc.x += o.x; acc.y += o.y; acc.z += o.z; acc.w += o.w;
+        b4 ob; ob[0] = (__bf16)o.x; ob[1] = (__bf16)o.y; ob[2] = (__bf16)o.z; ob[3] = (__bf16)o.w;
+        *reinterpret_cast<b4*>(dlogits + (long)r * V + 4 * c4) = ob;
+    };
+    int r = r0;
+    for (; r + 3 < r1; r += 4) {
+        float4 q[4];
+#pragma unroll
+        for (int u = 0; u < 4; ++u) q[u] = *reinterpret_cast<const float4*>(logits + (long)(r + u) * V + 4 * c4);
+#pragma unroll
+        for (int u = 0; u < 4; ++u) one(r + u, q[u], a[u]);
+    }
+    for (; r < r1; ++r) one(r, *reinterpret_cast<const float4*>(logits + (long)r * V + 4 * c4), a[0]);
+    if (!part) return;
+    float4 s;
+    s.x = (a[0].x + a[1].x) + (a[2].x + a[3].x); s.y = (a[0].y + a[1].y) + (a[2].y + a[3].y);
+    s.z = (a[0].z + a[1].z) + (a[2].z + a[3].z); s.w = (a[0].w + a[1].w) + (a[2].w + a[3].w);
+    *reinterpret_cast<float4*>(part + (long)blockIdx.y * V + 4 * c4) = s;
+}
+
 __global__ void ce_finish_kernel(const float* __restrict__ loss_rows, const int* __restrict__ correct_rows, int P, float* __restrict__ out) {
     __shared__ double s_l[256]; __shared__ int s_c[256];
     double s = 0.0; int c = 0;
diff --git a/show-attend-and-tell-pytorch-lightning_amd/decoder.py b/show-attend-and-tell-pytorch-lightning_amd/decoder.py
--- a/show-attend-and-tell-pytorch-lightning_amd/decoder.py
+++ b/show-attend-and-tell-pytorch-lightning_amd/decoder.py
@@ -167,35 +167,47 @@
 
     @staticmethod
     def backward(ctx, dlogits, dalphas):
-        lib = L.lib()
-        saved = list(ctx.saved_tensors)
-        ann, alphas = saved[0], saved[1]
-        it = iter(saved[2:])
-        params = [next(it) if present else None for present in ctx.present]
-        names = L.param_names(ctx.layers)
-        tens = dict(zip(names, params))
-        plan, dims = ctx.plan, ctx.dims
-        taken = set()
-
-        def gbuf(t):
-            if id(t) in taken:
-                return torch.empty_like(t)
-            taken.add(id(t))
-            return L.grad_buffer(t)
-
-        grads = {k: (None if t is None else gbuf(t)) for k, t in tens.items()}
-        dann = torch.empty_like(ann)
-        if dlogits is None:
-            dlogits = torch.zeros(plan.P, dims.V, dtype=torch.float32, device=ann.device)
-        dlogits = dlogits.contiguous()
-        dalphas = None if dalphas is None else dalphas.contiguous()
-        batch = L.DecoderBatch(ann=ann.data_ptr(), caps=ctx.caps.data_ptr(), lengths=plan.lengths.data_ptr(), prow=plan.prow.data_ptr(),
-                               src_row=plan.src_row.data_ptr(), step_offsets_host=plan.offsets_host.ctypes.data,
-                               teacher_host=ctx.teacher.ctypes.data)
-        w, g = _params_struct(tens, ctx.layers), _params_struct(grads, ctx.layers)
-        L.check(lib.sat_decoder_train_bwd(C.byref(dims), C.byref(w), C.byref(batch), L.ptr(dlogits), L.ptr(alphas), L.ptr(dalphas),
-                                          C.byref(g), L.ptr(dann), L.ptr(ctx.ws), ctx.ws_bytes, L.stream_ptr()), "sat_decoder_train_bwd")
-        return (dann, None, None, None, None, None, None, None, None, None, *[grads[k] for k in names])
+        dann, grads = _decoder_backward(ctx, dlogits, dalphas)
+        return (dann, None, None, None, None, None, None, None, None, None, *grads)
+
+
+def _decoder_backward(ctx, dlogits, dalphas, ce=None):
+    lib = L.lib()
+    saved = list(ctx.saved_tensors)
+    ann, alphas = saved[0], saved[1]
+    it = iter(saved[2:])
+    params = [next(it) if present else None for present in ctx.present]
+    names = L.param_names(ctx.layers)
+    tens = dict(zip(names, params))
+    plan, dims = ctx.plan, ctx.dims
+    taken = set()
+
+    def gbuf(t):
+        if id(t) in taken:
+            return torch.empty_like(t)
+        taken.add(id(t))
+        return L.grad_buffer(t)
+
+    grads = {k: (None if t is None else gbuf(t)) for k, t in tens.items()}
+    dann = torch.empty_like(ann)
+    dalphas = None if dalphas is None else dalphas.contiguous()
+    batch = L.DecoderBatch(ann=ann.data_ptr(), caps=ctx.caps.data_ptr(), lengths=plan.lengths.data_ptr(), prow=plan.prow.data_ptr(),
+                           src_row=plan.src_row.data_ptr(), step_offsets_host=plan.offsets_host.ctypes.data,
+                           teacher_host=ctx.teacher.ctypes.data)
+    w, g = _params_struct(tens, ctx.layers), _params_struct(grads, ctx.layers)
+    if ce is not None:
+        logits, targets, lse, smoothing, gscale = ce
+        dlogits_b = torch.empty(plan.P, dims.V, dtype=torch.bfloat16, device=ann.device)
+        L.check(lib.sat_decoder_train_bwd_ce(C.byref(dims), C.byref(w), C.byref(batch), L.ptr(logits), L.ptr(targets), L.ptr(lse), float(smoothing),
+                                             L.ptr(gscale), L.ptr(dlogits_b), L.ptr(alphas), L.ptr(dalphas), C.byref(g), L.ptr(dann), L.ptr(ctx.ws),
+                                             ctx.ws_bytes, L.stream_ptr()), "sat_decoder_train_bwd_ce")
+        return dann, [grads[k] for k in names]
+    if dlogits is None:
+        dlogits = torch.zeros(plan.P, dims.V, dtype=torch.float32, device=ann.device)
+    dlogits = dlogits.contiguous()
+    L.check(lib.sat_decoder_train_bwd(C.byref(dims), C.byref(w), C.byref(batch), L.ptr(dlogits), L.ptr(alphas), L.ptr(dalphas),
+                                      C.byref(g), L.ptr(dann), L.ptr(ctx.ws), ctx.ws_bytes, L.stream_ptr()), "sat_decoder_train_bwd")
+    return dann, [grads[k] for k in names]
 
 
 class LabelSmoothingFn(torch.autograd.Function):
@@ -228,6 +240,57 @@
         L.check(lib.sat_ce_label_smooth_bwd(L.ptr(logits), L.ptr(targets), L.ptr(lse), P, V, ctx.smoothing, L.ptr(g), L.ptr(dlogits),
                                             L.stream_ptr()), "sat_ce_label_smooth_bwd")
         return dlogits, None, None
+
+
+class PlainCtx:
+
+    def save_for_backward(self, *tensors):
+        self.saved_tensors = tuple(tensors)
+
+    def mark_non_differentiable(self, *tensors):
+        pass
+
+    def set_materialize_grads(self, value):
+        pass
+
+
+class DecoderLossFn(torch.autograd.Function):
+
+    last_handoff = None
+
+    @staticmethod
+    def forward(ctx, ann, caps_i32, targets_i32, smoothing, plan, teacher, deep, padding_idx, R, precision, embed_max_norm, dropout, *params):
+        dctx, cctx = PlainCtx(), PlainCtx()
+        logits, alphas = DecoderTrainFn.forward(dctx, ann, caps_i32, plan, teacher, deep, padding_idx, R, precision, embed_max_norm, dropout, *params)
+        loss, acc = LabelSmoothingFn.forward(cctx, logits, targets_i32, smoothing)
+        ctx.n_dec = len(dctx.saved_tensors)
+        ctx.save_for_backward(*dctx.saved_tensors, *cctx.saved_tensors)
+        dctx.saved_tensors = cctx.saved_tensors = None
+        ctx.dctx, ctx.cctx = dctx, cctx
+        ctx.mark_non_differentiable(acc)
+        ctx.set_materialize_grads(False)
+        return loss, acc, logits, alphas
+
+    @staticmethod
+    def backward(ctx, gloss, _gacc, glogits, dalphas):
+        if glogits is not None:
+            raise RuntimeError("DecoderLossFn: logits_packed is an output for reading; take gradients through DecoderTrainFn instead")
+        saved = tuple(ctx.saved_tensors)
+        dctx, cctx = ctx.dctx, ctx.cctx
+        dctx.saved_tensors, cctx.saved_tensors = saved[:ctx.n_dec], saved[ctx.n_dec:]
+        try:
+            handoff = gloss is not None and bool(L.lib().sat_decoder_loss_handoff(C.byref(dctx.dims)))
+            DecoderLossFn.last_handoff = handoff
+            if handoff:
+                logits, targets, lse = cctx.saved_tensors
+                g = gloss.reshape(1).to(torch.float32).contiguous()
+                dann, grads = _decoder_backward(dctx, None, dalphas, ce=(logits, targets, lse, cctx.smoothing, g))
+            else:
+                dlogits = None if gloss is None else LabelSmoothingFn.backward(cctx, gloss, None)[0]
+                dann, grads = _decoder_backward(dctx, dlogits, dalphas)
+        finally:
+            dctx.saved_tensors = cctx.saved_tensors = None
+        return (dann, None, None, None, None, None, None, None, None, None, None, None, *grads)
 
 
 class DoublyStochasticFn(torch.autograd.Function):
diff --git a/show-attend-and-tell-pytorch-lightning_amd/graph.py b/show-attend-and-tell-pytorch-lightning_amd/graph.py
--- a/show-attend-and-tell-pytorch-lightning_amd/graph.py
+++ b/show-attend-and-tell-pytorch-lightning_amd/graph.py
@@ -8,13 +8,7 @@
 from . import encoder as E
 
 
-class _Ctx:
-
-    def save_for_backward(self, *tensors):
-        self.saved_tensors = tuple(tensors)
-
-    def mark_non_differentiable(self, *tensors):
-        pass
+_Ctx = Dk.PlainCtx
 
 
 class _Entry:
@@ -107,20 +101,27 @@
             caps2 = caps.reshape(Bn * R, T)
             caps_i32 = caps2.to(dtype=torch.int32).contiguous()
             dec_params = model.param_list()
-            dctx = _Ctx()
-            logits, alphas = Dk.DecoderTrainFn.forward(dctx, ann_bld, caps_i32, plan, teacher, bool(hp.deep_output), model.pad_idx, R,
-                                                       int(model.sat_precision == "bf16"), getattr(hp, "embed_norm", None) or 0.0,
-                                                       model._dropout_args(None), *dec_params)
             targets = plan.pack(caps2[:, 1:].unsqueeze(-1)).squeeze(-1)
-            cctx, sctx = _Ctx(), _Ctx()
-            ce, acc = Dk.LabelSmoothingFn.forward(cctx, logits, targets.to(torch.int32), model.criterion.smoothing)
+            dec_args = (plan, teacher, bool(hp.deep_output), model.pad_idx, R, int(model.sat_precision == "bf16"), getattr(hp, "embed_norm", None) or 0.0,
+                        model._dropout_args(None))
+            dctx, cctx, sctx = _Ctx(), _Ctx(), _Ctx()
+            fused = model.sat_precision == "bf16"
+            if fused:
+                ce, acc, logits, alphas = Dk.DecoderLossFn.forward(dctx, ann_bld, caps_i32, targets.to(torch.int32), model.criterion.smoothing, *dec_args, *dec_params)
+            else:
+                logits, alphas = Dk.DecoderTrainFn.forward(dctx, ann_bld, caps_i32, *dec_args, *dec_params)
+                ce, acc = Dk.LabelSmoothingFn.forward(cctx, logits, targets.to(torch.int32), model.criterion.smoothing)
             model.criterion.last_accuracy = acc
             ds = Dk.DoublyStochasticFn.forward(sctx, alphas, float(hp.att_gamma))
             loss = ce + ds
             one = torch.ones((), dtype=torch.float32, device=img.device)
-            dlogits = Dk.LabelSmoothingFn.backward(cctx, one, None)[0]
             dalphas = Dk.DoublyStochasticFn.backward(sctx, one)[0]
-            douts = Dk.DecoderTrainFn.backward(dctx, dlogits, dalphas)
+            if fused:
+                douts = Dk.DecoderLossFn.backward(dctx, one, None, None, dalphas)
+                douts = douts[:1] + douts[3:]
+            else:
+                dlogits = Dk.LabelSmoothingFn.backward(cctx, one, None)[0]
+                douts = Dk.DecoderTrainFn.backward(dctx, dlogits, dalphas)
             dann = douts[0]
             grads = {}
 
diff --git a/show-attend-and-tell-pytorch-lightning_amd/model.py b/show-attend-and-tell-pytorch-lightning_amd/model.py
--- a/show-attend-and-tell-pytorch-lightning_amd/model.py
+++ b/show-attend-and-tell-pytorch-lightning_amd/model.py
@@ -446,16 +446,23 @@
             seed = int(torch.randint(0, 2 ** 62, (1,), generator=gen))
         return (p, pe, int(seed))
 
-    def train_decode(self, ann_bld, caps, lengths, epsilon=0, draw=None, with_loss=True, dropout_seed=None, teacher=None):
+    def train_decode(self, ann_bld, caps, lengths, epsilon=0, draw=None, with_loss=True, dropout_seed=None, teacher=None, fused_loss=False):
         B, R, T = caps.shape
         plan = Dk.PackPlan.cached(lengths.reshape(-1).cpu(), T, ann_bld.device)
         if teacher is None:
             teacher = plan.teacher_flags(float(epsilon), draw)
         caps2 = caps.reshape(B * R, T)
         caps_i32 = caps2.to(device=ann_bld.device, dtype=torch.int32).contiguous()
-        logits_packed, alphas = Dk.DecoderTrainFn.apply(ann_bld, caps_i32, plan, teacher, bool(self.hp.deep_output), self.pad_idx, R,
-                                                        int(getattr(self, "sat_precision", "fp32") == "bf16"), getattr(self.hp, "embed_norm", None) or 0.0,
-                                                        self._dropout_args(dropout_seed), *self.param_list())
+        dec_args = (plan, teacher, bool(self.hp.deep_output), self.pad_idx, R, int(getattr(self, "sat_precision", "fp32") == "bf16"),
+                    getattr(self.hp, "embed_norm", None) or 0.0, self._dropout_args(dropout_seed))
+        if with_loss and fused_loss:
+            targets_packed = plan.pack(caps2[:, 1:].to(ann_bld.device).unsqueeze(-1)).squeeze(-1)
+            ce, acc, logits_packed, alphas = Dk.DecoderLossFn.apply(ann_bld, caps_i32, targets_packed.to(torch.int32), self.criterion.smoothing, *dec_args,
+                                                                    *self.param_list())
+            self.criterion.last_accuracy = acc
+            ds = Dk.DoublyStochasticFn.apply(alphas, float(self.hp.att_gamma))
+            return dict(logits_packed=logits_packed, targets_packed=targets_packed, alphas=alphas, ce=ce, ds=ds, acc=acc, plan=plan)
+        logits_packed, alphas = Dk.DecoderTrainFn.apply(ann_bld, caps_i32, *dec_args, *self.param_list())
         targets_packed = plan.pack(caps2[:, 1:].to(ann_bld.device).unsqueeze(-1)).squeeze(-1)
         if not with_loss:
             return dict(logits_packed=logits_packed, targets_packed=targets_packed, alphas=alphas, plan=plan)
@@ -598,6 +605,11 @@
         return epsilon, gstep
 
     def _step_losses(self, batch, epsilon, teacher=None):
+        if getattr(self, "sat_precision", "fp32") == "bf16":
+            img, encoded_captions, lengths = batch
+            ann_bld, _ = self.encode(img)
+            res = self.train_decode(ann_bld, encoded_captions, lengths, float(epsilon), teacher=teacher, fused_loss=True)
+            return res["ce"] + res["ds"]
         lp, tp, alphas = self.train_batch(batch, epsilon, teacher=teacher)
         loss = self.criterion(lp.data, tp.data)
         loss = loss + Dk.DoublyStochasticFn.apply(alphas, float(self.hp.att_gamma))
```

New measurement: 32380 captions/s (median of 6 runs). About the same (+0.8%).
